# dmuley/sph-code

Measured on AMD Instinct MI355X. Metric: particle-steps/sec + achieved HBM GB/s, 10^6-particle 3D sphere, 1/2/4/8 GPUs, higher is better.
Workload: dtype f64

## Files before the change

sph-code_amd/csrc/sphx_api.hip:

```cpp
#include "sphx_internal.h"
#include <stdarg.h>
#include <stdlib.h>
#include <new>

int sphx_set_err(sphx_ctx* ctx, int code, const char* fmt, ...) {
    if (ctx) {
        va_list ap;
        va_start(ap, fmt);
        vsnprintf(ctx->err, sizeof(ctx->err), fmt, ap);
        va_end(ap);
    }
    return code;
}

void sphx_release(sphx_ctx* ctx, DevBuf& b) {
    for (size_t q = 0; q < ctx->allocs.size(); ++q)
        if (ctx->allocs[q] == b.p) { ctx->allocs[q] = ctx->allocs.back(); ctx->allocs.pop_back(); break; }
    if (b.p) (void)hipFree(b.p);
    b.p = nullptr;
    b.cap = 0;
}

int sphx_ensure(sphx_ctx* ctx, DevBuf& b, size_t bytes, hipStream_t in_use_on) {
    if (bytes == 0) bytes = 8;
    if (b.cap >= bytes) return SPHX_OK;
    if (b.p) {
        HIPCHK(hipStreamSynchronize(in_use_on));
        sphx_release(ctx, b);
    }
    size_t want = bytes + bytes / 8 + 256;
    hipError_t e = hipMalloc(&b.p, want);
    if (e != hipSuccess) {
        b.p = nullptr;
        return sphx_set_err(ctx, SPHX_E_NOMEM, "hipMalloc(%zu) failed: %s", want, hipGetErrorString(e));
    }
    b.cap = want;
    ctx->allocs.push_back(b.p);
    return SPHX_OK;
}

static void default_constants(sphx_constants* c) {
    c->k_B = 1.380649e-23;
    c->amu = 1.66053906892e-27;
    c->m_h = 1.0008 * c->amu;
    c->m_0 = 31.622776601683793 * 1.989e30;
    c->dt_0 = 60. * 60. * 24. * 365. * 250000.;
    c->max_age = 3e7 * 60. * 60. * 24. * 365.;
    c->pos_clamp = 1e11 * 149597870700.0;
    c->solar_luminosity = 3.846e26;
    c->c = 299792458.0;
}

extern "C" int sphx_version(void) { return 100; }

extern "C" const char* sphx_build_info(void) { return "gfx950 experiments=0"; }
extern "C" const char* sphx_tunables(const sphx_ctx* ctx) { return ctx ? ctx->tunables : ""; }

extern "C" int sphx_host_alloc(void** out, size_t bytes) {
    if (!out) return SPHX_E_ARG;
    *out = nullptr;
    if (bytes == 0) bytes = 8;
    if (hipHostMalloc(out, bytes, hipHostMallocDefault) != hipSuccess) {
        (void)hipGetLastError();
        *out = nullptr;
        return SPHX_E_NOMEM;
    }
    return SPHX_OK;
}
extern "C" int sphx_host_free(void* p) {
    if (p && hipHostFree(p) != hipSuccess) return SPHX_E_HIP;
    return SPHX_OK;
}

static hipError_t sphx_stream_create(hipStream_t* st, int side) {
    int least = 0, greatest = 0;
    if (hipDeviceGetStreamPriorityRange(&least, &greatest) != hipSuccess) return hipStreamCreateWithFlags(st, hipStreamNonBlocking);
    return hipStreamCreateWithPriority(st, hipStreamNonBlocking, side ? least : greatest);
}

extern "C" int sphx_create(sphx_ctx** out, int device) {
    if (!out) return SPHX_E_ARG;
    *out = nullptr;
    int count = 0;
    if (hipGetDeviceCount(&count) != hipSuccess || count <= 0 || device < 0 || device >= count) {
        fprintf(stderr, "sphx_create: no usable HIP device %d (found %d). libsphx has no CPU path.\n",
                device, count);
        return SPHX_E_HIP;
    }
    sphx_ctx* ctx = new (std::nothrow) sphx_ctx();
    if (!ctx) return SPHX_E_NOMEM;
    ctx->device = device;
    memset(&ctx->stats, 0, sizeof(ctx->stats));
    memset(&ctx->grid, 0, sizeof(ctx->grid));
    default_constants(&ctx->cst);
    auto env = [&](const char* name) -> const char* {
        const char* e = getenv(name);
        if (e) {
            const size_t used = strlen(ctx->tunables);
            snprintf(ctx->tunables + used, sizeof(ctx->tunables) - used, "%s%s=%s", used ? " " : "", name, e);
        }
        return e;
    };
    if (const char* e = env("SPHX_RSCALE")) { double v = atof(e); if (v >= 1.0) ctx->rscale = v; }
    if (const char* e = env("SPHX_CELL")) { double v = atof(e); if (v > 0.0) ctx->cell_factor = v; }
    if (const char* e = env("SPHX_RSCALE_BUILD")) { double v = atof(e); if (v >= 1.0) ctx->rscale_build = v; }
    if (const char* e = env("SPHX_VERLET")) ctx->use_verlet = atoi(e) != 0;
    if (const char* e = env("SPHX_BLOB")) ctx->use_blob = atoi(e) != 0;
    if (const char* e = env("SPHX_BLOB_CURVE")) ctx->blob_curve = atoi(e);
    if (const char* e = env("SPHX_KNN_GROUP")) ctx->use_group = atoi(e) != 0;
    if (const char* e = env("SPHX_HCLIP")) { double v = atof(e); if (v > 1.0) ctx->h_clip_factor = v; }
    if (const char* e = env("SPHX_TIMING_DETAIL")) ctx->timing_detail = atoi(e) != 0;
    if (const char* e = env("SPHX_MAX_CELLS")) { long long v = atoll(e); if (v > 0) ctx->max_cells = v; }
    if (const char* e = env("SPHX_CELL_FEEDBACK")) ctx->cell_feedback = atoi(e) != 0;
    if (const char* e = env("SPHX_CELL_FB_HI")) ctx->cell_fb_hi = atof(e);
    if (const char* e = env("SPHX_CELL_FB_LO")) ctx->cell_fb_lo = atof(e);
    if (const char* e = env("SPHX_DRAG_LDS")) ctx->drag_lds = atoi(e) != 0;
    if (const char* e = env("SPHX_BLOB_SPLIT")) ctx->blob_split_on = atoi(e) != 0;
    if (const char* e = env("SPHX_SPECIES_FUSED")) ctx->species_fused = atoi(e) != 0;
    if (const char* e = env("SPHX_SPECIES_LDS")) ctx->species_lds = atoi(e) != 0;
    if (const char* e = env("SPHX_HINT_DISTRUST")) ctx->distrust_mode = atoi(e);
    if (const char* e = env("SPHX_OUTLIER_LEVELS")) ctx->olev_mode = atoi(e);
    if (const char* e = env("SPHX_BOX_SIGMAS")) { double v = atof(e); if (v >= 1.0) ctx->box_sigmas = v; }
    if (const char* e = env("SPHX_GRAV_KERNEL")) ctx->grav_per_thread = atoi(e) == 0;
    if (const char* e = env("SPHX_GRAV_ORDER")) { int v = atoi(e); if (v == 1 || v == 2) ctx->grav_order = v; }
    if (const char* e = env("SPHX_GRAV_WS")) { int v = atoi(e); if (v >= 1 && v <= 4) ctx->grav_ws = v; }
    if (const char* e = env("SPHX_LDS")) ctx->use_lds = atoi(e) != 0;
    if (const char* e = env("SPHX_BLOB_SLOTS")) ctx->blob_slots = atoi(e);
    if (const char* e = env("SPHX_BLOB_WGS")) {
        int cus = 256;
        (void)hipDeviceGetAttribute(&cus, hipDeviceAttributeMultiprocessorCount, ctx->device);
        if (atoi(e) > 0) ctx->blob_grid = ((cus * atoi(e) + 7) / 8) * 8;
    }
    bool ok = hipSetDevice(device) == hipSuccess &&
              sphx_stream_create(&ctx->stream, 0) == hipSuccess &&
              hipHostMalloc((void**)&ctx->pinned, sizeof(PinnedLayout), hipHostMallocDefault) == hipSuccess;
    ctx->own_stream = ctx->stream;
    for (int i = 0; ok && i < 10; ++i) ok = hipEventCreate(&ctx->ev[i]) == hipSuccess;
    for (int r = 0; ok && r < 3; ++r)
        for (int i = 0; ok && i < 10; ++i) ok = hipEventCreate(&ctx->evring[r][i]) == hipSuccess;
    for (int r = 0; ok && r < 2; ++r)
        ok = hipEventCreateWithFlags(&ctx->lag_bev[r], hipEventDisableTiming) == hipSuccess &&
             hipEventCreateWithFlags(&ctx->lag_hev[r], hipEventDisableTiming) == hipSuccess;
    if (ok) ok = sphx_stream_create(&ctx->side_stream, 1) == hipSuccess &&
                 hipEventCreateWithFlags(&ctx->ev_join, hipEventDisableTiming) == hipSuccess &&
                 hipEventCreateWithFlags(&ctx->ev_perm, hipEventDisableTiming) == hipSuccess;
    if (ok) ok = sphx_ensure(ctx, ctx->scal, SC_NSLOTS * 8) == SPHX_OK &&
                 hipMemsetAsync(ctx->scal.p, 0, SC_NSLOTS * 8, ctx->stream) == hipSuccess &&
                 sphx_ensure(ctx, ctx->badc, (size_t)BADC_BUCKETS * BADC_STRIDE * sizeof(u64)) == SPHX_OK &&
                 hipMemsetAsync(ctx->badc.p, 0, (size_t)BADC_BUCKETS * BADC_STRIDE * sizeof(u64), ctx->stream) == hipSuccess;
    if (!ok) {
        fprintf(stderr, "sphx_create: HIP initialisation failed on device %d\n", device);
        delete ctx;
        return SPHX_E_HIP;
    }
    *out = ctx;
    return SPHX_OK;
}

extern "C" void sphx_destroy(sphx_ctx* ctx) {
    if (!ctx) return;
    (void)hipSetDevice(ctx->device);
    if (ctx->stream) (void)hipStreamSynchronize(ctx->stream);
    for (void* p : ctx->allocs) (void)hipFree(p);
    for (int i = 0; i < 10; ++i)
        if (ctx->ev[i]) (void)hipEventDestroy(ctx->ev[i]);
    for (StageTimer* t : {&ctx->arb_t, &ctx->rad_t, &ctx->cool_t})
        for (int i = 0; i < 5; ++i)
            if (t->ev[i]) (void)hipEventDestroy(t->ev[i]);
    for (int r = 0; r < 3; ++r)
        for (int i = 0; i < 10; ++i)
            if (ctx->evring[r][i]) (void)hipEventDestroy(ctx->evring[r][i]);
    for (int r = 0; r < 2; ++r) {
        if (ctx->lag_bev[r]) (void)hipEventDestroy(ctx->lag_bev[r]);
        if (ctx->lag_hev[r]) (void)hipEventDestroy(ctx->lag_hev[r]);
    }
    if (ctx->pinned) (void)hipHostFree(ctx->pinned);
    if (ctx->olev_ev) (void)hipEventDestroy(ctx->olev_ev);
    if (ctx->ev_join) (void)hipEventDestroy(ctx->ev_join);
    if (ctx->ev_perm) (void)hipEventDestroy(ctx->ev_perm);
    if (ctx->side_stream) (void)hipStreamDestroy(ctx->side_stream);
    if (ctx->own_stream) (void)hipStreamDestroy(ctx->own_stream);
    delete ctx;
}

extern "C" const char* sphx_last_error(const sphx_ctx* ctx) { return ctx ? ctx->err : "null context"; }

extern "C" int sphx_set_constants(sphx_ctx* ctx, const sphx_constants* c) {
    if (!ctx || !c) return SPHX_E_ARG;
    ctx->cst = *c;
    return SPHX_OK;
}
extern "C" int sphx_set_tuning(sphx_ctx* ctx, double rscale, double cell_factor) {
    if (!ctx) return SPHX_E_ARG;
    if (rscale > 0.0) {
        if (rscale < 1.0) return sphx_set_err(ctx, SPHX_E_ARG, "rscale %g < 1", rscale);
        ctx->rscale = rscale;
    }
    if (cell_factor > 0.0) ctx->cell_factor = cell_factor;
    return SPHX_OK;
}
extern "C" int sphx_set_incremental(sphx_ctx* ctx, int verlet, double rscale_build) {
    if (!ctx) return SPHX_E_ARG;
    ctx->use_verlet = verlet != 0;
    if (!ctx->use_verlet) ctx->list_valid = false;
    if (rscale_build > 0.0) {
        if (rscale_build < 1.0) return sphx_set_err(ctx, SPHX_E_ARG, "rscale_build %g < 1", rscale_build);
        ctx->rscale_build = rscale_build;
    }
    return SPHX_OK;
}
extern "C" int sphx_get_constants(const sphx_ctx* ctx, sphx_constants* c) {
    if (!ctx || !c) return SPHX_E_ARG;
    *c = ctx->cst;
    return SPHX_OK;
}

static int upload(sphx_ctx* ctx, DevBuf& b, const void* host, size_t bytes) {
    SPHX_TRY(sphx_ensure(ctx, b, bytes));
    HIPCHK(hipMemcpyAsync(b.p, host, bytes, hipMemcpyHostToDevice, ctx->stream));
    return SPHX_OK;
}
static int download(sphx_ctx* ctx, void* host, const void* dev, size_t bytes) {
    if (!host) return SPHX_OK;
    HIPCHK(hipMemcpyAsync(host, dev, bytes, hipMemcpyDeviceToHost, ctx->stream));
    return SPHX_OK;
}
int sphx_upload_f64(sphx_ctx* ctx, const CopyF64* t, int nt) {
    for (int i = 0; i < nt; ++i)
        if (t[i].host)
            HIPCHK(hipMemcpyAsync(const_cast<void*>(t[i].dev), t[i].host, t[i].count * sizeof(double), hipMemcpyHostToDevice, ctx->stream));
    return SPHX_OK;
}
int sphx_download_f64(sphx_ctx* ctx, const CopyF64* t, int nt) {
    for (int i = 0; i < nt; ++i)
        if (t[i].host && t[i].dev && t[i].count > 0)
            HIPCHK(hipMemcpyAsync(const_cast<void*>(t[i].host), t[i].dev, t[i].count * sizeof(double), hipMemcpyDeviceToHost, ctx->stream));
    return SPHX_OK;
}

int StageTimer::begin(sphx_ctx* ctx) {
    for (int i = 0; i < 5; ++i)
        if (!ev[i]) HIPCHK(hipEventCreate(&ev[i]));
    for (int i = 0; i < 4; ++i) ms[i] = 0.0;
    return mark(ctx, 0);
}
int StageTimer::mark(sphx_ctx* ctx, int i) {
    HIPCHK(hipEventRecord(ev[i], ctx->stream));
    return SPHX_OK;
}
int StageTimer::end(sphx_ctx* ctx) {
    for (int i = 0; i < 4; ++i) {
        float t = 0.f;
        HIPCHK(hipEventElapsedTime(&t, ev[i], ev[i + 1]));
        ms[i] = t;
    }
    return SPHX_OK;
}
static int last_timing(sphx_ctx* ctx, StageTimer sphx_ctx::*t, double ms[4]) {
    if (!ctx || !ms) return SPHX_E_ARG;
    for (int i = 0; i < 4; ++i) ms[i] = (ctx->*t).ms[i];
    return SPHX_OK;
}
extern "C" int sphx_arb_last_timing(sphx_ctx* ctx, double ms[4]) { return last_timing(ctx, &sphx_ctx::arb_t, ms); }
extern "C" int sphx_rad_last_timing(sphx_ctx* ctx, double ms[4]) { return last_timing(ctx, &sphx_ctx::rad_t, ms); }
extern "C" int sphx_cool_last_timing(sphx_ctx* ctx, double ms[4]) { return last_timing(ctx, &sphx_ctx::cool_t, ms); }

extern "C" int sphx_neighbors(sphx_ctx* ctx, int64_t n, int k, const double* points, double dist,
                              double eps, int64_t* idx, double* dist_out, int64_t* nontriv,
                              double* h) {
    (void)eps;
// ... 245 lines not shown
static int step_cell_hint(sphx_ctx* ctx, int64_t n, double* cell_hint) {
    *cell_hint = 0.0;
    if (ctx->step_count == 0) return SPHX_OK;
    const double* hs;
    if (ctx->lag_hvalid[ctx->lag_hslot]) {
        HIPCHK(hipEventSynchronize(ctx->lag_halias[ctx->lag_hslot] ? ctx->lag_halias[ctx->lag_hslot]
                                                                     : ctx->lag_hev[ctx->lag_hslot]));
        hs = ctx->pinned->lag[ctx->lag_hslot].hs;
        const u64* sv = (const u64*)hs;
        for (int q = 0; q < 10; ++q) ctx->knn_lag[q] = sv[(SC_NFAILQ - SC_HSUM) + q];
        ctx->knn_lag_valid = true;
    } else {
        HIPCHK(hipMemcpyAsync(ctx->pinned->hsum, ctx->scal.as<double>() + SC_HSUM, sizeof(ctx->pinned->hsum),
                              hipMemcpyDeviceToHost, ctx->stream));
        HIPCHK(hipStreamSynchronize(ctx->stream));
        hs = ctx->pinned->hsum;
    }
    const double hmean = hs[3] > 0.0 ? hs[0] / hs[3] : 0.0;
    if (hmean > 0.0 && isfinite(hmean)) {
        *cell_hint = ctx->cell_factor * sphx_cell_feedback(ctx, n) * hmean;
        ctx->h_clip = ctx->h_clip_factor * hmean;
    }
    return SPHX_OK;
}

static int step_search(sphx_ctx* ctx, int k, double dist, hipEvent_t* ev) {
    const int64_t n = ctx->n;
    if (ctx->use_verlet) SPHX_TRY(sphx_clamp(ctx, n, ctx->st));
    SPHX_TRY(sphx_ensure(ctx, ctx->nbr, (size_t)k * ctx->npad * sizeof(int)));
    if (ctx->use_verlet && ctx->list_valid && ctx->list_n == n && ctx->list_k == k) {
        StateArrays& r = ctx->st;
        HIPCHK(hipEventRecord(ev[1], ctx->stream));
        int64_t nfail = 0;
        SPHX_TRY(sphx_knn_refresh(ctx, n, k, r.x.as<double>(), r.y.as<double>(), r.z.as<double>(),
                                  ctx->nbr.as<int>(), r.hprev.as<double>(), &nfail));
        if (nfail == 0) {
            ctx->stats.refresh_steps++;
            return SPHX_OK;
        }
        ctx->list_valid = false;
    }
    double cell_hint = 0.0;
    SPHX_TRY(step_cell_hint(ctx, n, &cell_hint));
    {
        StateArrays& r = ctx->st;
        const bool blob = ctx->use_blob && !ctx->use_verlet;
        GridBuildOpts g;
        g.lagged = true;
        g.alias_ev = ev[1];
        g.sort_cells_later = blob;
        g.count_curve = blob && ctx->side_stream && ctx->ev_perm;
        if (!ctx->use_verlet) { g.clamp_vel[0] = r.vx.as<double>(); g.clamp_vel[1] = r.vy.as<double>(); g.clamp_vel[2] = r.vz.as<double>(); }
        SPHX_TRY(sphx_build_grid(ctx, n, k, r.x.as<double>(), r.y.as<double>(), r.z.as<double>(), cell_hint, g));
        if (blob) SPHX_TRY(sphx_build_blob_order(ctx, n, true));
    }
    const bool split = ctx->side_stream && !ctx->use_verlet;
    SPHX_TRY(sphx_permute_state(ctx, n, split, ev[1]));
    StateArrays& r = ctx->st;
    KnnIn in;
    in.xs = r.x.as<double>(); in.ys = r.y.as<double>(); in.zs = r.z.as<double>();
    in.id = r.id.as<int>(); in.inv = ctx->inv.as<int>();
    in.rsearch = r.hprev.as<double>();
    in.hinted = ctx->step_count > 0 && !ctx->use_verlet;
    in.lag_external = true;
    in.rscale = ctx->rscale;
    in.rbound = dist;
    KnnOut o;
    o.nbr = ctx->nbr.as<int>();
    o.h_sorted = r.hprev.as<double>();
    o.idx64 = nullptr; o.dist = nullptr; o.nontriv = nullptr; o.h_by_id = nullptr;
    if (ctx->use_verlet) {
        SPHX_TRY(sphx_ensure(ctx, ctx->list64, (size_t)n * 64 * sizeof(int)));
        SPHX_TRY(sphx_ensure(ctx, ctx->dref, (size_t)n * sizeof(double)));
        o.list64 = ctx->list64.as<int>();
        o.dref = ctx->dref.as<double>();
        in.rscale = ctx->rscale_build;
    }
    SPHX_TRY(sphx_knn(ctx, n, k, in, o));
    if (split) HIPCHK(hipStreamWaitEvent(ctx->stream, ctx->ev_perm, 0));
    if (ctx->use_verlet) {
        SPHX_TRY(sphx_save_list_positions(ctx, n, r.x.as<double>(), r.y.as<double>(), r.z.as<double>()));
        ctx->list_valid = true;
        ctx->list_n = n;
        ctx->list_k = k;
    }
    ctx->stats.rebuild_steps++;
    return SPHX_OK;
}

static int step_h_sums_out(sphx_ctx* ctx, int64_t n, const double* h, hipStream_t stream) {
    SPHX_TRY(sphx_hsum(ctx, n, h, stream));
    const int hsl = ctx->lag_hslot ^ 1;
    HIPCHK(hipMemcpyAsync(ctx->pinned->lag[hsl].hs, ctx->scal.as<double>() + SC_HSUM,
                          (SC_KGDBG + 2 - SC_HSUM + 1) * sizeof(double), hipMemcpyDeviceToHost, stream));
    HIPCHK(hipEventRecord(ctx->lag_hev[hsl], stream));
    ctx->lag_halias[hsl] = nullptr;
    ctx->lag_hvalid[hsl] = true;
    ctx->lag_hslot = hsl;
    return SPHX_OK;
}

static int step_sums(sphx_ctx* ctx, int k, hipEvent_t* ev, hipEvent_t search_end, bool detail) {
    const int64_t n = ctx->n;
    StateArrays& s = ctx->st;
    const bool pairwise = ctx->visc_mode == 1 && !ctx->loop_forms;
    const bool fork = ctx->qorder && ctx->use_lds && !ctx->loop_forms && ctx->side_stream;
    if (fork) HIPCHK(hipStreamWaitEvent(ctx->side_stream, search_end, 0));
    else SPHX_TRY(step_h_sums_out(ctx, n, s.hprev.as<double>(), ctx->stream));
    if (ctx->qorder && ctx->use_lds) SPHX_TRY(sphx_blob_translate(ctx, n, k));
    const bool species = ctx->s > 0 && ctx->fun_id.p;
    if (ctx->loop_forms) {
        if (ctx->drag || species)
            SPHX_TRY(sphx_prep(ctx, n, prep_in_of_state(s), pairwise, ctx->stream));
        if (detail) HIPCHK(hipEventRecord(ev[3], ctx->stream));
        SPHX_TRY(sphx_loop_step_sums(ctx, n, k, ctx->loop_d));
        if (detail) HIPCHK(hipEventRecord(ev[9], ctx->stream));
        if (species) SPHX_TRY(sphx_step_species(ctx, n, k));
        if (detail) HIPCHK(hipEventRecord(ev[4], ctx->stream));
        if (detail) HIPCHK(hipEventRecord(ev[5], ctx->stream));
    } else {
        SPHX_TRY(sphx_prep(ctx, n, prep_in_of_state(s), pairwise, fork ? ctx->side_stream : ctx->stream));
        if (fork) {
            HIPCHK(hipEventRecord(ctx->ev_join, ctx->side_stream));
            HIPCHK(hipStreamWaitEvent(ctx->stream, ctx->ev_join, 0));
            SPHX_TRY(step_h_sums_out(ctx, n, s.hprev.as<double>(), ctx->side_stream));
        }
        if (detail) HIPCHK(hipEventRecord(ev[3], ctx->stream));
        const bool sp_fused = species && ctx->species_fused && ctx->species_lds && ctx->use_lds && ctx->qorder && ctx->blob_lists &&
                              !ctx->map_perm && ctx->sp == 16 && ctx->s <= 16 && k <= SPHX_MAX_K;
        if (sp_fused) {
            const int S = ctx->s;
            SPHX_TRY(sphx_ensure(ctx, ctx->rho, (size_t)n * sizeof(double)));
            SPHX_TRY(sphx_ensure(ctx, ctx->rhod, (size_t)n * sizeof(double)));
            SPHX_TRY(sphx_ensure(ctx, ctx->nden, (size_t)n * sizeof(double)));
            SPHX_TRY(sphx_ensure(ctx, ctx->G, (size_t)n * 3 * sizeof(double)));
            SPHX_TRY(sphx_ensure(ctx, ctx->ha, (size_t)n * 3 * sizeof(double)));
            SPHX_TRY(sphx_ensure(ctx, ctx->F, (size_t)n * S * sizeof(double)));
            if (ctx->agb_on) {
                SPHX_TRY(sphx_ensure(ctx, ctx->Zmet, (size_t)n * sizeof(double)));
                SPHX_TRY(sphx_ensure(ctx, ctx->agb_dust, (size_t)n * S * sizeof(double)));
            }
            SPHX_TRY(sphx_blob_density_species(ctx, n, k, true, S, ctx->fun_id.as<double>(), s.id.as<int>(),
                                               s.m.as<double>(), ctx->F.as<double>(), ctx->Zmet.as<double>(),
                                               ctx->agb_dust.as<double>(), (ctx->agb_on && ctx->Zmet.p && ctx->agb_dust.p) ? 1 : 0));
        } else {
            SPHX_TRY(sphx_pass_density(ctx, n, k, true));
        }
        if (detail) HIPCHK(hipEventRecord(ev[9], ctx->stream));
        if (species && !sp_fused) SPHX_TRY(sphx_step_species(ctx, n, k));
        if (detail) HIPCHK(hipEventRecord(ev[4], ctx->stream));
        if (ctx->visc_mode == 1) {
            SPHX_TRY(sphx_pass_visc_pw(ctx, n, k, s.m.as<double>()));
        } else {
            SPHX_TRY(sphx_pass_pi(ctx, n, k, s.hprev.as<double>(), s.ptype.as<double>()));
            if (detail) HIPCHK(hipEventRecord(ev[5], ctx->stream));
            SPHX_TRY(sphx_pass_visc(ctx, n, k, s.m.as<double>()));
        }
    }
    if (ctx->drag)
        SPHX_TRY(sphx_pass_drag(ctx, n, k, s.m.as<double>(), s.ptype.as<double>(), s.mgm.as<double>(), s.mcs.as<double>()));
    return SPHX_OK;
}

static int one_step(sphx_ctx* ctx, int k, double dist, int first, double fixed_dt, bool call_first, bool call_last) {
    const int64_t n = ctx->n;
    const int ring = (int)(ctx->step_count % 3);
    hipEvent_t* ev = ctx->evring[ring];
    const bool detail = ctx->timing_detail;
    ctx->ev_detail[ring] = detail;
    const bool rec0 = detail || call_first, rec7 = detail || call_last;
    ctx->ev_has07[ring] = (rec0 ? 1 : 0) | (rec7 ? 2 : 0) | (ctx->visc_mode == 1 && !ctx->loop_forms ? 4 : 0);
    ctx->map_perm = nullptr;
    ctx->qorder = nullptr;
    ctx->blob_lists = false;
    ctx->blob_split_valid = false;
    ctx->pass_part = 0;
    ctx->nbr_api_valid = false;
    if (rec0) HIPCHK(hipEventRecord(ev[0], ctx->stream));
    SPHX_TRY(step_search(ctx, k, dist, ev));
    HIPCHK(hipEventRecord(ev[2], ctx->stream));
    SPHX_TRY(step_sums(ctx, k, ev, ev[2], detail));
    if (detail) HIPCHK(hipEventRecord(ev[6], ctx->stream));
    StateArrays& s = ctx->st;
    if (ctx->gravity) {
        SPHX_TRY(sphx_ensure(ctx, ctx->grav, (size_t)n * 3 * sizeof(double)));
        double* eps = ctx->scal.as<double>() + SC_GRAV_EPS;
        SPHX_TRY(sphx_median(ctx, n, s.hprev.as<double>(), eps));
        if (ctx->gravity == 1)
            SPHX_TRY(sphx_gravity_launch(ctx, n, s.x.as<double>(), s.y.as<double>(), s.z.as<double>(), 1,
                                         s.m.as<double>(), eps, 0.0, ctx->grav_G, nullptr, ctx->grav.as<double>()));
        else
            SPHX_TRY(sphx_gravity_tree_launch(ctx, n, s.x.as<double>(), s.y.as<double>(), s.z.as<double>(),
                                              s.m.as<double>(), ctx->grav_ws, eps, 0.0, ctx->grav_G, nullptr,
                                              ctx->grav.as<double>()));
    }
    if (detail) HIPCHK(hipEventRecord(ev[8], ctx->stream));
    SPHX_TRY(sphx_integrate(ctx, n, 1, first, fixed_dt));
    if (rec7) HIPCHK(hipEventRecord(ev[7], ctx->stream));
    ctx->step_count++;
    return SPHX_OK;
}

static int collect_stats(sphx_ctx* ctx, int ring) {
    if (!(ctx->ev_pending & (1u << ring))) return SPHX_OK;
    ctx->ev_pending &= ~(1u << ring);
    hipEvent_t* ev = ctx->evring[ring];
    const int has = ctx->ev_has07[ring];
    HIPCHK(hipEventSynchronize((has & 2) ? ev[7] : ev[2]));
    sphx_stats& st = ctx->stats;
    float ms[7] = {0.f, 0.f, 0.f, 0.f, 0.f, 0.f, 0.f};
    HIPCHK(hipEventElapsedTime(&ms[1], ev[1], ev[2]));
    st.ms_search += ms[1];
    st.steps += 1;
    st.search_steps += 1;
    st.n = ctx->n;
    if (!ctx->ev_detail[ring]) return SPHX_OK;
    float tot;
    HIPCHK(hipEventElapsedTime(&tot, ev[0], ev[7]));
    HIPCHK(hipEventElapsedTime(&ms[0], ev[0], ev[1]));
    st.ms_grid += ms[0]; st.ms_total += tot;
    for (int i = 2; i < 6; ++i) {
        if ((has & 4) && i >= 4) break;
        HIPCHK(hipEventElapsedTime(&ms[i], ev[i], ev[i + 1]));
    }
    if (has & 4) HIPCHK(hipEventElapsedTime(&ms[5], ev[4], ev[6]));
    st.ms_prep += ms[2];
    float mg = 0.f, mi = 0.f;
    HIPCHK(hipEventElapsedTime(&mg, ev[6], ev[8]));
    HIPCHK(hipEventElapsedTime(&mi, ev[8], ev[7]));
    ms[6] = mi;
    st.ms_gravity += mg;
    {
        float md = 0.f, msp = 0.f;
        HIPCHK(hipEventElapsedTime(&md, ev[3], ev[9]));
        HIPCHK(hipEventElapsedTime(&msp, ev[9], ev[4]));
        ms[3] = md;
        st.ms_species += msp;
    }
    st.ms_density += ms[3]; st.ms_pi += ms[4]; st.ms_visc += ms[5]; st.ms_integrate += ms[6];
    st.detail_steps += 1;
    return SPHX_OK;
}

extern "C" int sphx_step(sphx_ctx* ctx, int nsteps, int k, double dist, int first, double fixed_dt) {
    if (!ctx) return SPHX_E_ARG;
    if (!ctx->has_state) return sphx_set_err(ctx, SPHX_E_STATE, "sphx_step before sphx_state_upload");
    if (k < 1 || k > SPHX_MAX_K) return sphx_set_err(ctx, SPHX_E_ARG, "N_NEIGH=%d not in 1..%d", k, SPHX_MAX_K);
    if (nsteps < 1) return sphx_set_err(ctx, SPHX_E_ARG, "nsteps=%d < 1", nsteps);
    HIPCHK(hipSetDevice(ctx->device));
    if (!(dist > 0.0) || !isfinite(dist)) dist = 0.0;
    ctx->k = k;
    const bool per_call = !ctx->timing_detail;
    if (per_call) HIPCHK(hipEventRecord(ctx->ev[8], ctx->stream));
    for (int it = 0; it < nsteps; ++it) {
        const int ring = (int)(ctx->step_count % 3);
        SPHX_TRY(collect_stats(ctx, ring));
        SPHX_TRY(one_step(ctx, k, dist, first && it == 0, fixed_dt, false, false));
        ctx->ev_pending |= 1u << ring;
        SPHX_TRY(collect_stats(ctx, (ring + 1) % 3));
    }
    if (per_call) HIPCHK(hipEventRecord(ctx->ev[9], ctx->stream));
    HIPCHK(hipMemcpyAsync(ctx->pinned->scal, ctx->scal.p, SC_NSLOTS * 8, hipMemcpyDeviceToHost, ctx->stream));
    HIPCHK(hipStreamSynchronize(ctx->stream));
    for (int r = 0; r < 3; ++r) SPHX_TRY(collect_stats(ctx, (int)((ctx->step_count + r) % 3)));
    if (per_call) {
        float tot = 0.f;
        HIPCHK(hipEventElapsedTime(&tot, ctx->ev[8], ctx->ev[9]));
        ctx->stats.ms_total += tot;
    }
    const u64* sc = ctx->pinned->scal;
    memcpy(&ctx->dt_last, &sc[SC_DT], sizeof(double));
    ctx->stats.candidates = (int64_t)sc[SC_CAND];
    ctx->stats.retries = (int64_t)sc[SC_RETRY];
    ctx->stats.fallback_queries = (int64_t)(u32)sc[SC_NFAILQ];
    ctx->stats.short_rows = (int64_t)sc[SC_SHORT];
    SPHX_TRY(sphx_badc_read(ctx));
    return SPHX_OK;
}

extern "C" int sphx_state_download(sphx_ctx* ctx, double* pos, double* vel, double* accel,
                                   double* E_internal, double* T, double* sizes, double* rho,
                                   double* nden, double* visc_heat, double* dt_last) {
    if (!ctx) return SPHX_E_ARG;
    if (!ctx->has_state) return sphx_set_err(ctx, SPHX_E_STATE, "no state uploaded");
    HIPCHK(hipSetDevice(ctx->device));
    const int64_t n = ctx->n;
    const size_t nb = (size_t)n * sizeof(double);
    StateArrays& s = ctx->st;
    const int* id = s.id.as<int>();
    SPHX_TRY(sphx_ensure(ctx, ctx->out_a, 3 * nb));
    double* stage = ctx->out_a.as<double>();
    struct V3 { double* host; DevBuf *a, *b, *c; };
    V3 v3[] = {{pos, &s.x, &s.y, &s.z}, {vel, &s.vx, &s.vy, &s.vz}, {accel, &s.ax, &s.ay, &s.az}};
    for (V3& v : v3) {
        if (!v.host) continue;
        SPHX_TRY(sphx_soa3_to_aos_by_id(ctx, n, id, v.a->as<double>(), v.b->as<double>(), v.c->as<double>(), stage));
        SPHX_TRY(download(ctx, v.host, stage, 3 * nb));
        HIPCHK(hipStreamSynchronize(ctx->stream));
    }
    struct V1 { double* host; const double* dev; };
    const bool stepped = ctx->step_count > 0;
    V1 v1[] = {{E_internal, s.E.as<double>()}, {T, s.T.as<double>()}, {sizes, s.hprev.as<double>()},
               {rho, stepped ? ctx->rho.as<double>() : nullptr},
               {nden, stepped ? ctx->nden.as<double>() : nullptr},
               {visc_heat, stepped ? ctx->vh.as<double>() : nullptr}};
    for (V1& v : v1) {
        if (!v.host) continue;
        if (!v.dev) { memset(v.host, 0, nb); continue; }
        SPHX_TRY(sphx_scatter_rows_by_id(ctx, n, 1, id, v.dev, stage));
        SPHX_TRY(download(ctx, v.host, stage, nb));
        HIPCHK(hipStreamSynchronize(ctx->stream));
    }
    if (dt_last) *dt_last = ctx->dt_last;
    return SPHX_OK;
}

int sphx_agb_table_set(sphx_ctx* ctx, int S, int nspl, const int32_t* ntx, const int32_t* nty, const double* tx, const double* ty,
                       const double* coeffs, const int32_t* mapto, double divisor, const double* mu_specie, double solar_mass) {
    ctx->agb_on = false;
    if (nspl == 0) return SPHX_OK;
    if (S < 7 || S > AGB_MAX_SPEC) return sphx_set_err(ctx, SPHX_E_ARG, "AGB table: %d species (7..%d)", S, AGB_MAX_SPEC);
    if (!ntx || !nty || !tx || !ty || !coeffs || !mapto || !mu_specie)
        return sphx_set_err(ctx, SPHX_E_ARG, "AGB table: NULL argument");
    if (nspl < 1 || nspl > AGB_MAX_SPL) return sphx_set_err(ctx, SPHX_E_ARG, "AGB table: %d splines", nspl);
    if (!(divisor != 0.0)) return sphx_set_err(ctx, SPHX_E_ARG, "AGB table: divisor is 0");
    HIPCHK(hipSetDevice(ctx->device));
    AgbTable& t = ctx->agb;
    t.nspl = nspl; t.nspec = S;
// ... 155 lines not shown
```

sph-code_amd/csrc/sphx_blob.h:

```cpp
#pragma once
#include "sphx_internal.h"
#include "sphx_pair.h"
#include "sphx_settled.h"

#ifndef BLOB_P
#define BLOB_P 128
#endif
#define BLOB_T (2 * BLOB_P)
#define LPP SPHX_SUM_PARTS
#define PASS_T (BLOB_P * LPP)
#ifndef BLOB_S
#define BLOB_S 960
#endif
#ifndef DEDUP_PRIO
#define DEDUP_PRIO 2
#endif
#ifndef BLOB_STAGE_PRIO
#define BLOB_STAGE_PRIO 1
#endif
#ifndef PASS_MINW
#define PASS_MINW 4
#endif
#define BLOB_PROBES 96
#define SLOT_NONE 0xFFFFu
// ... 3 lines not shown
typedef unsigned short u16;

__device__ __forceinline__ Q4 lload4(const double2* img, int s, int c2) {
    const double2 lo = img[(2 * c2) * BLOB_S + s];
    const double2 hi = img[(2 * c2 + 1) * BLOB_S + s];
    return Q4{lo.x, lo.y, hi.x, hi.y};
}
struct Q8 { Q4 lo, hi; };
__device__ __forceinline__ Q8 lload8(const double2* img, int s) { return Q8{lload4(img, s, 0), lload4(img, s, 1)}; }
template <class Rec>
__device__ __forceinline__ Q8 gload8(const Rec* r) {
    const double* q = reinterpret_cast<const double*>(r);
    return Q8{gload4(q), gload4(q + 4)};
}
__device__ __forceinline__ double sqrt_mid(double x) {
    const double y = __builtin_amdgcn_rsq(x);
    double g = x * y;
    double h = 0.5 * y;
    const double r = __builtin_fma(-h, g, 0.5);
    g = __builtin_fma(g, r, g);
    h = __builtin_fma(h, r, h);
    const double d0 = __builtin_fma(-g, g, x);
    g = __builtin_fma(d0, h, g);
    const double d1 = __builtin_fma(-g, g, x);
    g = __builtin_fma(d1, h, g);
    return x > 0.0 ? g : 0.0;
}
struct SqrtMid { __device__ __forceinline__ double operator()(double x) const { return sqrt_mid(x); } };

__device__ __forceinline__ double pair_swap(double v) {
    const long long b = __double_as_longlong(v);
    const int lo = __builtin_amdgcn_update_dpp(0, (int)b, 0xB1, 0xF, 0xF, true);
    const int hi = __builtin_amdgcn_update_dpp(0, (int)(b >> 32), 0xB1, 0xF, 0xF, true);
    return __longlong_as_double(((long long)hi << 32) | (unsigned)lo);
}
__device__ __forceinline__ double pair_swap2(double v) {
    const long long b = __double_as_longlong(v);
    const int lo = __builtin_amdgcn_update_dpp(0, (int)b, 0x4E, 0xF, 0xF, true);
    const int hi = __builtin_amdgcn_update_dpp(0, (int)(b >> 32), 0x4E, 0xF, 0xF, true);
    return __longlong_as_double(((long long)hi << 32) | (unsigned)lo);
}
__device__ __forceinline__ double group_total(double acc) {
    acc = acc + pair_swap(acc);
    if (LPP == 4) acc = acc + pair_swap2(acc);
    return acc;
}
__device__ __forceinline__ double group_max(double v) {
    v = fmax(v, pair_swap(v));
    if (LPP == 4) v = fmax(v, pair_swap2(v));
    return v;
}
template <class S>
__device__ __forceinline__ void group_total_fields(S& s) {
    constexpr int NF = sizeof(S) / sizeof(double);
    static_assert(sizeof(S) == NF * sizeof(double), "a struct of doubles");
    double f[NF];
    __builtin_memcpy(f, &s, sizeof(S));
#pragma unroll
    for (int q = 0; q < NF; ++q) f[q] = group_total(f[q]);
    __builtin_memcpy(&s, f, sizeof(S));
}

#define NSTAGE ((BLOB_S + PASS_T - 1) / PASS_T)
#define NB (8 / LPP)
#define KPAD(k) ((((k) + 7) / 8) * 8)
#define IMG_BYTES(per_slot, k) ((size_t)BLOB_S * (per_slot) + (size_t)KPAD(k) * BLOB_P * sizeof(u16))

template <int NSIDE, class Rec>
__device__ __forceinline__ void stage(double2* img, double* side, u16* tile, const Rec* __restrict__ rec,
                                      const double* __restrict__ g0, int g0_stride,
                                      const double* __restrict__ g1, int g1_stride,
                                      const int* __restrict__ uq, const u16* __restrict__ slot16, int npad,
                                      int k, int b) {
    __builtin_amdgcn_s_setprio(BLOB_STAGE_PRIO);
    int ju[NSTAGE];
#pragma unroll
    for (int r = 0; r < NSTAGE; ++r) {
        const int s = threadIdx.x + r * PASS_T;
        ju[r] = (s < BLOB_S) ? uq[s] : -1;
    }
    const int pieces = KPAD(k) * (BLOB_P / 8);
    for (int q = threadIdx.x; q < pieces; q += PASS_T) {
        const int kk = q / (BLOB_P / 8), c = q % (BLOB_P / 8);
        uint4 v = make_uint4(0xFFFFFFFFu, 0xFFFFFFFFu, 0xFFFFFFFFu, 0xFFFFFFFFu);
        if (kk < k) v = *reinterpret_cast<const uint4*>(slot16 + (size_t)kk * npad + (size_t)b * BLOB_P + c * 8);
        *reinterpret_cast<uint4*>(tile + kk * BLOB_P + c * 8) = v;
    }
    double2 c[NSTAGE][4];
    double e0[NSTAGE], e1[NSTAGE];
#pragma unroll
    for (int r = 0; r < NSTAGE; ++r) {
        const int j = ju[r] < 0 ? 0 : ju[r];
        const double2* g = reinterpret_cast<const double2*>(&rec[j]);
        c[r][0] = g[0]; c[r][1] = g[1]; c[r][2] = g[2]; c[r][3] = g[3];
        e0[r] = (NSIDE > 0) ? g0[(size_t)j * g0_stride] : 0.0;
        e1[r] = (NSIDE > 1) ? g1[(size_t)j * g1_stride] : 0.0;
    }
#pragma unroll
    for (int r = 0; r < NSTAGE; ++r) {
        const int s = threadIdx.x + r * PASS_T;
        if (ju[r] >= 0) {
            if (NSIDE == 2) c[r][3].y = e0[r];
            img[0 * BLOB_S + s] = c[r][0]; img[1 * BLOB_S + s] = c[r][1];
            img[2 * BLOB_S + s] = c[r][2]; img[3 * BLOB_S + s] = c[r][3];
            if (NSIDE == 1) side[s] = e0[r];
            if (NSIDE == 2) side[s] = e1[r];
        }
    }
    __builtin_amdgcn_s_setprio(0);
}

__device__ __forceinline__ void load_slots(unsigned (&sl)[NB], const u16* tile, int m0, int half, int t) {
#pragma unroll
    for (int u = 0; u < NB; ++u) sl[u] = tile[(LPP * (m0 + u) + half) * BLOB_P + t];
}
__device__ __forceinline__ bool all_staged(const unsigned (&sl)[NB]) {
    unsigned worst = sl[0];
#pragma unroll
    for (int u = 1; u < NB; ++u) worst = worst > sl[u] ? worst : sl[u];
    return __ballot(worst >= SLOT_OVER) == 0ull;
}


struct BlobSel { const int* list; const int* cnt; int mode; };
__device__ __forceinline__ int blob_sel_count(const BlobSel& s, int nblk) {
    if (!s.list) return nblk;
    return (s.mode == 1) ? s.cnt[0] : (s.mode == 2) ? s.cnt[1] : s.cnt[0] + s.cnt[1];
}
__device__ __forceinline__ int blob_sel_at(const BlobSel& s, int bi, int count) {
    const int q = xcd_block(bi, count);
    return s.list ? s.list[q + (s.mode == 2 ? s.cnt[0] : 0)] : q;
}
BlobSel sphx_blob_sel(sphx_ctx* ctx, int part);

int sphx_blob_grid(sphx_ctx* ctx, int nblk);
int sphx_lds_opt_in(sphx_ctx* ctx, const void* kernel, size_t bytes);

#define BLOB_KERNEL __global__ __launch_bounds__(PASS_T, PASS_MINW) void
#define BLOB_COMMON int n, int npad, int k, int nblk, const int* __restrict__ nbr, const u16* __restrict__ slot16, \
                    const int* __restrict__ uniq, const int* __restrict__ qorder
template <class Kern, class... Rest>
static int blob_launch(sphx_ctx* ctx, Kern kern, int per_slot, size_t extra, int64_t n, int k, Rest... rest) {
    const int64_t npad = sphx_pad64(n);
    const int nblk = (int)((npad + BLOB_P - 1) / BLOB_P);
    SPHX_TRY(sphx_lds_opt_in(ctx, reinterpret_cast<const void*>(kern), IMG_BYTES(per_slot, SPHX_MAX_K) + extra));
    hipLaunchKernelGGL(kern, dim3(sphx_blob_grid(ctx, nblk)), dim3(PASS_T), IMG_BYTES(per_slot, k) + extra, ctx->stream, (int)n,
                       (int)npad, k, nblk, ctx->nbr.as<int>(), ctx->slot16.as<u16>(), ctx->uniq.as<int>(), ctx->qorder, rest...);
    HIPCHK(hipGetLastError());
    return SPHX_OK;
}

template <class P, class = void> struct BlobSettles { static constexpr bool value = false; };
template <class P> struct BlobSettles<P, decltype((void)P::SETTLES)> { static constexpr bool value = P::SETTLES; };
template <class P, class = void> struct BlobSaturates { static constexpr bool value = false; };
template <class P> struct BlobSaturates<P, decltype((void)P::SATURATES)> { static constexpr bool value = P::SATURATES; };
enum { BLOB_CNT_BLOBS_SETTLED = 0, BLOB_CNT_WAVES_SATURATED = 1 };
struct BlobSides { const double* g0 = nullptr; int s0 = 0; const double* g1 = nullptr; int s1 = 0; };

template <int NSIDE>
struct BlobLds {
    static __device__ __forceinline__ double2* img() { extern __shared__ double2 img[]; return img; }
    static __device__ __forceinline__ double* side() { return reinterpret_cast<double*>(img() + 4 * BLOB_S); }
    static __device__ __forceinline__ u16* tile() { return reinterpret_cast<u16*>(side() + (NSIDE ? BLOB_S : 0)); }
};

template <bool FAST, bool CLIP, class P>
__device__ __forceinline__ void blob_batch(const P& ps, typename P::Sums& a, double (&out)[NB], const unsigned (&sl)[NB],
                                           const int* __restrict__ jp, size_t colstep, const typename P::Row& row) {
    typedef BlobLds<P::NSIDE> L;
    typename P::Nb f[NB];
#pragma unroll
    for (int u = 0; u < NB; ++u) {
        if (FAST || sl[u] < SLOT_OVER) f[u] = ps.staged(L::img(), L::side(), (int)sl[u], jp + u * colstep);
        else if (sl[u] == SLOT_OVER) f[u] = ps.global(jp[u * colstep]);
        else f[u] = P::none(row);
    }
    if (FAST) __builtin_amdgcn_sched_barrier(0);
#pragma unroll
    for (int u = 0; u < NB; ++u) {
        out[u] = 0.0;
        if (!FAST && sl[u] == SLOT_NONE) continue;
        out[u] = ps.template term<CLIP>(a, f[u], row);
    }
}
template <class P>
__device__ __forceinline__ void blob_batch_any(const P& ps, int clip, typename P::Sums& a, double (&out)[NB],
                                               const unsigned (&sl)[NB], const int* __restrict__ jp, size_t colstep,
                                               const typename P::Row& row) {
    const bool fast = all_staged(sl);
    if constexpr (P::CLIPS) {
        if (fast && !clip) blob_batch<true, false>(ps, a, out, sl, jp, colstep, row);
        else if (fast) blob_batch<true, true>(ps, a, out, sl, jp, colstep, row);
        else if (!clip) blob_batch<false, false>(ps, a, out, sl, jp, colstep, row);
        else blob_batch<false, true>(ps, a, out, sl, jp, colstep, row);
    } else {
        if (fast) blob_batch<true, false>(ps, a, out, sl, jp, colstep, row);
        else blob_batch<false, false>(ps, a, out, sl, jp, colstep, row);
    }
}
template <bool FAST, class P>
__device__ __forceinline__ void blob_batch_short(const P& ps, double (&out)[NB], const unsigned (&sl)[NB],
                                                 const int* __restrict__ jp, size_t colstep, const typename P::Row& row) {
    typedef BlobLds<P::NSIDE> L;
    typename P::Vel f[NB];
#pragma unroll
    for (int u = 0; u < NB; ++u) {
        if (FAST || sl[u] < SLOT_OVER) f[u] = P::short_staged(L::img(), (int)sl[u]);
        else if (sl[u] == SLOT_OVER) f[u] = ps.short_global(jp[u * colstep]);
        else f[u] = P::short_none(row);
    }
#pragma unroll
    for (int u = 0; u < NB; ++u) {
        out[u] = 0.0;
        if (!FAST && sl[u] == SLOT_NONE) continue;
        out[u] = P::term_short(f[u], row);
    }
}
struct RowAhead { int i, o; unsigned first; double own; };
template <class P>
__device__ __forceinline__ RowAhead blob_row_ahead(const P& ps, int i, int p, int n, const u16* __restrict__ slot16,
                                                   const int* __restrict__ omap) {
    RowAhead r;
    r.i = i;
    r.o = (p < n) ? (omap ? omap[i] : i) : 0x7FFFFFFF;
    r.first = (p < n) ? slot16[p] : SLOT_NONE;
    r.own = ps.own(i);
    return r;
}
template <int T>
__device__ __forceinline__ bool block_all_at_barrier(bool mine, unsigned round) {
    __shared__ int verdict[2][T / 64];
    static_assert(T / 64 == 8, "eight waves: read as two 16-B pieces");
    int* v = verdict[round & 1];
    const int wave_all = __ballot(!mine) == 0ull;
    if ((threadIdx.x & 63) == 0) v[threadIdx.x >> 6] = wave_all;
    __syncthreads();
    const int4 lo = *reinterpret_cast<const int4*>(v), hi = *reinterpret_cast<const int4*>(v + 4);
    const int all = (lo.x & lo.y) & (lo.z & lo.w) & (hi.x & hi.y) & (hi.z & hi.w);
    return __builtin_amdgcn_readfirstlane(all) != 0;
}
template <int T>
__device__ __forceinline__ void block_add_count(unsigned v, u64* dst) {
    __shared__ unsigned sm[T / 64];
    if ((threadIdx.x & 63) == 0) sm[threadIdx.x >> 6] = v;
    __syncthreads();
    if (threadIdx.x == 0) {
        unsigned r = 0;
        for (int w = 0; w < T / 64; ++w) r += sm[w];
        if (r) atomicAdd(dst, (u64)r);
    }
}
template <class P>
__device__ __forceinline__ void blob_row_point(const P& ps, typename P::Row& row, const int* __restrict__ nbr, int p,
                                               int t) {
    typedef BlobLds<P::NSIDE> L;
    const unsigned sl0 = L::tile()[t];
    if (sl0 < SLOT_OVER) P::row_point(row, ps.staged(L::img(), L::side(), (int)sl0, nbr + p));
    else if (sl0 == SLOT_OVER) P::row_point(row, ps.global(nbr[p]));
}

template <class P>
__device__ __forceinline__ void blob_pass(const P& ps, int n, int npad, int k, int nblk, const int* __restrict__ nbr,
                                          const u16* __restrict__ slot16, const int* __restrict__ uniq,
                                          const int* __restrict__ qorder, int clip, const int* __restrict__ omap,
                                          int n_active, u64* ct_bits, const BlobSel& sel, u64* counts = nullptr) {
    static_assert(P::PER_SLOT == 64 + (P::NSIDE ? 8 : 0), "image bytes per slot: the record and one side value");
    constexpr bool SETTLES = BlobSettles<P>::value, SATURATES = BlobSaturates<P>::value;
    static_assert(!SATURATES || LPP == 4, "sphx_wave_saturated: a row's lanes are one nibble of the wave's mask");
    typedef BlobLds<P::NSIDE> L;
    const BlobSides sd = ps.sides();
    const int t = threadIdx.x / LPP, half = threadIdx.x & (LPP - 1);
    u64 my_ct = SPHX_CT_NONE;
    unsigned blobs_settled = 0, waves_saturated = 0;
    const int nsel = blob_sel_count(sel, nblk);
    const int stride = gridDim.x;
    auto particle_of = [&](int bq) -> int {
        const int pq = blob_sel_at(sel, bq, nsel) * BLOB_P + t;
        return (pq < n) ? qorder[pq] : 0;
    };
    auto nothing_left = [&](const RowAhead& r) -> bool {
        return !(r.o < n_active) || sphx_row_settled(r.own, r.first != SLOT_NONE, true);
    };
    RowAhead cur{0, 0x7FFFFFFF, SLOT_NONE, 0.0};
    int i_next = 0;
    bool blob_settled = false;
    unsigned round = 0;
    if constexpr (SETTLES) {
        if ((int)blockIdx.x < nsel)
            cur = blob_row_ahead(ps, particle_of(blockIdx.x), blob_sel_at(sel, blockIdx.x, nsel) * BLOB_P + t, n, slot16, omap);
        if ((int)blockIdx.x + stride < nsel) i_next = particle_of(blockIdx.x + stride);
        blob_settled = block_all_at_barrier<PASS_T>(nothing_left(cur), round++);
    }
    for (int bi = blockIdx.x; bi < nsel; bi += stride) {
        const int b = blob_sel_at(sel, bi, nsel);
        const int p = b * BLOB_P + t;
        int i, o;
        bool settled = false;
        auto fetch_ahead = [&]() {
            if constexpr (SETTLES) {
                if (bi + stride < nsel) {
                    cur = blob_row_ahead(ps, i_next, blob_sel_at(sel, bi + stride, nsel) * BLOB_P + t, n, slot16, omap);
                    if (bi + 2 * stride < nsel) i_next = particle_of(bi + 2 * stride);
                }
            }
        };
        if constexpr (SETTLES) {
            i = cur.i; o = cur.o;
            settled = sphx_row_settled(cur.own, cur.first != SLOT_NONE, o < n_active);
            if (blob_settled) {
                fetch_ahead();
                if (settled && !half) ps.settle(o);
                ++blobs_settled;
                blob_settled = block_all_at_barrier<PASS_T>(nothing_left(cur), round++);
                continue;
            }
        } else {
            i = (p < n) ? qorder[p] : 0;
        }
        stage<P::NSIDE>(L::img(), L::side(), L::tile(), ps.rec, sd.g0, sd.s0, sd.g1, sd.s1, uniq + (size_t)b * BLOB_S,
                        slot16, npad, k, b);
        typename P::Row row = ps.load_row(i);
        if constexpr (!SETTLES) o = (p < n) ? (omap ? omap[i] : i) : 0x7FFFFFFF;
        ps.load_out(row, o, o < n_active);
        if constexpr (SETTLES) fetch_ahead();
        __syncthreads();
        if (o < n_active) {
            if (SETTLES && __ballot(!settled) == 0ull) {
                if constexpr (SETTLES) { if (!half) ps.settle(o); }
            } else {
                if constexpr (P::ROW_FROM_LIST) blob_row_point(ps, row, nbr, p, t);
                typename P::Sums a{};
                double mx = 0.0;
                if (P::wanted(row)) {
                    const int nm = KPAD(k) / LPP;
                    unsigned sl[NB];
                    load_slots(sl, L::tile(), 0, half, t);
                    bool short_form = false;
                    bool short_used = false;
                    for (int m0 = 0; m0 < nm; m0 += NB) {
                        unsigned cur_sl[NB];
#pragma unroll
                        for (int u = 0; u < NB; ++u) cur_sl[u] = sl[u];
                        if (m0 + NB < nm) load_slots(sl, L::tile(), m0 + NB, half, t);
                        double out[NB];
                        const int* jp = nbr + ((size_t)(LPP * m0 + half) * npad + p);
                        if constexpr (SATURATES) {
                            if (__builtin_expect(short_form, false)) {
                                short_used = true;
                                if (all_staged(cur_sl)) blob_batch_short<true>(ps, out, cur_sl, jp, LPP * (size_t)npad, row);
                                else blob_batch_short<false>(ps, out, cur_sl, jp, LPP * (size_t)npad, row);
                            } else {
                                blob_batch_any(ps, clip, a, out, cur_sl, jp, LPP * (size_t)npad, row);
                                short_form = sphx_wave_saturated(__ballot(P::saturated(a)), __ballot(true));
                            }
                        } else {
                            blob_batch_any(ps, clip, a, out, cur_sl, jp, LPP * (size_t)npad, row);
                        }
                        if (P::VOTES) {
#pragma unroll
                            for (int u = 0; u < NB; ++u) mx = fmax(mx, out[u]);
                        }
                    }
                    if (SATURATES && short_used) ++waves_saturated;
                }
                group_total_fields(a);
                if (P::VOTES) mx = group_max(mx);
                if (!half) {
                    const u64 cb = ps.finish(a, mx, row, i, o);
                    my_ct = cb < my_ct ? cb : my_ct;
                }
            }
        }
        if constexpr (SETTLES) blob_settled = block_all_at_barrier<PASS_T>(nothing_left(cur), round++);
        else __syncthreads();
    }
    if (P::VOTES) block_min_vote<PASS_T>(my_ct, ct_bits);
    if constexpr (SETTLES) {
        if (counts && threadIdx.x == 0 && blobs_settled) atomicAdd(counts + BLOB_CNT_BLOBS_SETTLED, (u64)blobs_settled);
    }
    if constexpr (SATURATES) {
        if (counts) block_add_count<PASS_T>(waves_saturated, counts + BLOB_CNT_WAVES_SATURATED);
    }
}
```

sph-code_amd/csrc/sphx_blob.hip:

```cpp
#include "sphx_blob.h"
#include "sphx_wave.h"
#pragma clang fp contract(off)
#include <float.h>
#include <stdlib.h>
#include <stdio.h>
#ifndef BLOB_PI_SATURATES
#define BLOB_PI_SATURATES 1
#endif

#define DD_TAB 2048
#define DD_PROBES 64
__device__ __forceinline__ unsigned dd_hash(int j) { return ((unsigned)j * 2654435761u) >> 21; }

__global__ __launch_bounds__(BLOB_T) void blob_dedup_kernel(int n, int npad, int k, int slots,
                                                            const int* __restrict__ nbr, u16* slot16,
                                                            int* uniq, const int* __restrict__ qorder,
                                                            const int* __restrict__ omap, int n_active,
                                                            unsigned char* bclass) {
    __builtin_amdgcn_s_setprio(DEDUP_PRIO);
    extern __shared__ u16 dd_tile[];
    __shared__ int key[DD_TAB];
    __shared__ u16 slot_of[DD_TAB];
    __shared__ int wave_tot[BLOB_T / 64];
    const int b = xcd_block(blockIdx.x, gridDim.x);
    const int t = threadIdx.x >> 1, half = threadIdx.x & 1;
    const int p = b * BLOB_P + t;
    for (int q = threadIdx.x; q < DD_TAB; q += BLOB_T) key[q] = -1;
    __syncthreads();
    {
        const int nm = (k + 1) >> 1;
        const bool live = p < n;
        int jn[DD_BATCH];
#pragma unroll
        for (int u = 0; u < DD_BATCH; ++u) {
            const int kk = 2 * u + half;
            jn[u] = (kk < k && live) ? nbr[(size_t)kk * npad + p] : -1;
        }
        for (int m0 = 0; m0 < nm; m0 += DD_BATCH) {
            int jb[DD_BATCH];
#pragma unroll
            for (int u = 0; u < DD_BATCH; ++u) {
                jb[u] = jn[u];
                const int kk = 2 * (m0 + DD_BATCH + u) + half;
                jn[u] = (kk < k && live) ? nbr[(size_t)kk * npad + p] : -1;
            }
            unsigned hb[DD_BATCH];
            int eb[DD_BATCH];
#pragma unroll
            for (int u = 0; u < DD_BATCH; ++u) {
                hb[u] = dd_hash(jb[u] < 0 ? 0 : jb[u]);
                eb[u] = key[hb[u]];
            }
#pragma unroll
            for (int u = 0; u < DD_BATCH; ++u)
                if (jb[u] >= 0 && eb[u] == -1) {
                    const int old = atomicCAS(&key[hb[u]], -1, jb[u]);
                    eb[u] = (old == -1) ? jb[u] : old;
                }
#pragma unroll
            for (int u = 0; u < DD_BATCH; ++u) {
                const int kk = 2 * (m0 + u) + half;
                if (kk >= k) continue;
                const int j = jb[u];
                unsigned s = SLOT_NONE;
                if (j >= 0) {
                    unsigned h = hb[u];
                    s = SLOT_OVER;
                    if (eb[u] == j) {
                        s = h;
                    } else {
                        for (int probe = 1; probe < DD_PROBES; ++probe) {
                            h = (h + 1) & (DD_TAB - 1);
                            int e = key[h];
                            if (e == -1) {
                                e = atomicCAS(&key[h], -1, j);
                                if (e == -1) e = j;
                            }
                            if (e == j) { s = h; break; }
                        }
                    }
                }
                dd_tile[kk * BLOB_P + t] = (u16)s;
            }
        }
    }
    __syncthreads();
    constexpr int EPT = DD_TAB / BLOB_T;
    const int e0 = threadIdx.x * EPT;
    int cnt = 0;
#pragma unroll
    for (int q = 0; q < EPT; ++q) cnt += key[e0 + q] != -1;
    const int incl = wave_scan_incl(cnt);
    const int lane = threadIdx.x & 63, wv = threadIdx.x >> 6;
    if (lane == 63) wave_tot[wv] = incl;
    __syncthreads();
    int base = incl - cnt, total = 0;
#pragma unroll
    for (int w = 0; w < BLOB_T / 64; ++w) {
        const int tw = wave_tot[w];
        if (w < wv) base += tw;
        total += tw;
    }
    int* uq = uniq + (size_t)b * BLOB_S;
    int needs_ghost = 0;
#pragma unroll
    for (int q = 0; q < EPT; ++q) {
        const int j = key[e0 + q];
        if (j != -1) {
            slot_of[e0 + q] = (u16)(base < slots ? base : SLOT_OVER);
            if (base < slots) uq[base] = j;
            ++base;
            if (bclass && omap[j] >= n_active) needs_ghost = 1;
        }
    }
    for (int q = (total < slots ? total : slots) + threadIdx.x; q < BLOB_S; q += BLOB_T) uq[q] = -1;
    __syncthreads();
    const int pieces = k * (BLOB_P / 8);
    for (int q = threadIdx.x; q < pieces; q += BLOB_T) {
        u16* src = dd_tile + q * 8;
        const int kk = q / (BLOB_P / 8), c = q % (BLOB_P / 8);
        unsigned v[8];
#pragma unroll
        for (int u = 0; u < 8; ++u) {
            const unsigned e = src[u];
            v[u] = e < DD_TAB ? (unsigned)slot_of[e] : e;
            if (v[u] == SLOT_OVER) needs_ghost = 1;
        }
        if ((size_t)b * BLOB_P + c * 8 < (size_t)npad)
            *reinterpret_cast<uint4*>(slot16 + (size_t)kk * npad + (size_t)b * BLOB_P + c * 8) =
                make_uint4(v[0] | (v[1] << 16), v[2] | (v[3] << 16), v[4] | (v[5] << 16), v[6] | (v[7] << 16));
    }
    if (bclass) {
        const int owned_q = (half == 0 && p < n && omap[qorder[p]] < n_active) ? 1 : 0;
        const int any_owned = __syncthreads_or(owned_q);
        const int any_ghost = __syncthreads_or(needs_ghost);
        if (threadIdx.x == 0) bclass[b] = (unsigned char)(!any_owned ? 2 : (any_ghost ? 1 : 0));
    }
}

#define SPLIT_T 1024
__global__ __launch_bounds__(SPLIT_T) void blob_split_kernel(int nblk, const unsigned char* __restrict__ bclass, int* list,
                                                             int* cnt) {
    __shared__ int wsum[2][SPLIT_T / 64];
    const int per = (nblk + SPLIT_T - 1) / SPLIT_T;
    const int b0 = threadIdx.x * per, b1 = (b0 + per < nblk) ? b0 + per : nblk;
    int c0 = 0, c1 = 0;
    for (int b = b0; b < b1; ++b) { const int c = bclass[b]; c0 += c == 0; c1 += c == 1; }
    const int i0 = wave_scan_incl(c0), i1 = wave_scan_incl(c1);
    const int lane = threadIdx.x & 63, wv = threadIdx.x >> 6;
    if (lane == 63) { wsum[0][wv] = i0; wsum[1][wv] = i1; }
    __syncthreads();
    int o0 = i0 - c0, o1 = i1 - c1, t0 = 0, t1 = 0;
    for (int w = 0; w < SPLIT_T / 64; ++w) {
        if (w < wv) { o0 += wsum[0][w]; o1 += wsum[1][w]; }
        t0 += wsum[0][w]; t1 += wsum[1][w];
    }
    for (int b = b0; b < b1; ++b) {
        const int c = bclass[b];
        if (c == 0) list[o0++] = b;
        else if (c == 1) list[t0 + o1++] = b;
    }
    if (threadIdx.x == 0) { cnt[0] = t0; cnt[1] = t1; cnt[2] = nblk - t0 - t1; }
}

int sphx_blob_translate(sphx_ctx* ctx, int64_t n, int k) {
    const int64_t npad = sphx_pad64(n);
    const int nblk = (int)((npad + BLOB_P - 1) / BLOB_P);
    SPHX_TRY(sphx_ensure(ctx, ctx->slot16, (size_t)k * npad * sizeof(u16) + 512));
    SPHX_TRY(sphx_ensure(ctx, ctx->uniq, (size_t)nblk * BLOB_S * sizeof(int)));
    int slots = ctx->blob_slots;
    if (slots < 1) slots = 1;
    if (slots > BLOB_S) slots = BLOB_S;
    const bool split = ctx->map_perm != nullptr && ctx->blob_split_on;
    unsigned char* bclass = nullptr;
    ctx->blob_split_valid = false;
    if (split) {
        SPHX_TRY(sphx_ensure(ctx, ctx->blob_class, (size_t)nblk));
        SPHX_TRY(sphx_ensure(ctx, ctx->blob_split, ((size_t)nblk + 4) * sizeof(int)));
        bclass = ctx->blob_class.as<unsigned char>();
    }
    hipLaunchKernelGGL(blob_dedup_kernel, dim3(nblk), dim3(BLOB_T), (size_t)k * BLOB_P * sizeof(u16), ctx->stream, (int)n, (int)npad, k, slots,
                       ctx->nbr.as<int>(), ctx->slot16.as<u16>(), ctx->uniq.as<int>(), ctx->qorder, ctx->map_perm,
                       ctx->map_nactive, bclass);
    if (split) {
        int* list = ctx->blob_split.as<int>();
        hipLaunchKernelGGL(blob_split_kernel, dim3(1), dim3(SPLIT_T), 0, ctx->stream, nblk, bclass, list, list + (size_t)nblk);
        ctx->blob_split_valid = true;
        ctx->blob_split_nblk = nblk;
    }
    HIPCHK(hipGetLastError());
    ctx->blob_lists = true;
    return SPHX_OK;
}


struct DensityPass {
    typedef RecA Rec;
    typedef DensAcc Sums;
    static constexpr int NSIDE = 0, PER_SLOT = 64;
    static constexpr bool CLIPS = true, VOTES = false, ROW_FROM_LIST = true;
    const RecA* __restrict__ rec;
    double *rho_s, *rho, *rhod, *nden, *G, *ha;
    struct Row { double xr, yr, zr, hi2, ci, Ai; };
    typedef Q8 Nb;
    __device__ __forceinline__ BlobSides sides() const { return {}; }
    __device__ __forceinline__ Row load_row(int i) const {
        const Q8 s = gload8(&rec[i]);
        return Row{s.lo.a, s.lo.b, s.lo.c, s.lo.d, -6.0 * s.hi.a, s.hi.c};
    }
    __device__ __forceinline__ static void load_out(Row&, int, bool) {}
    __device__ __forceinline__ static void row_point(Row& r, const Nb& f) { r.xr = f.lo.a; r.yr = f.lo.b; r.zr = f.lo.c; }
    __device__ __forceinline__ static bool wanted(const Row&) { return true; }
    __device__ __forceinline__ Nb staged(const double2* img, const double*, int s, const int*) const {
        return lload8(img, s);
    }
    __device__ __forceinline__ Nb global(int j) const { return gload8(&rec[j]); }
    __device__ __forceinline__ static Nb none(const Row& r) { return Nb{Q4{r.xr, r.yr, r.zr, 0.0}, Q4{0.0, 0.0, 0.0, 0.0}}; }
    template <bool CLIP>
    __device__ __forceinline__ double term(Sums& a, const Nb& f, const Row& r) const {
        return density_term<SqrtMid>(a, f.lo, f.hi, r.xr, r.yr, r.zr, r.hi2, r.ci, r.Ai, CLIP);
    }
    __device__ __forceinline__ u64 finish(const Sums& a, double, const Row&, int i, int o) const {
        rho[o] = a.rho; rhod[o] = a.rd; nden[o] = a.n;
        rho_s[i] = a.rho;
        if (G) { G[3 * (size_t)o + 0] = -a.gx; G[3 * (size_t)o + 1] = -a.gy; G[3 * (size_t)o + 2] = -a.gz; }
        ha[3 * (size_t)o + 0] = -a.gx / a.rho;
        ha[3 * (size_t)o + 1] = -a.gy / a.rho;
        ha[3 * (size_t)o + 2] = -a.gz / a.rho;
        return SPHX_CT_NONE;
    }
};
BLOB_KERNEL blob_density_kernel(BLOB_COMMON, int clip, const int* __restrict__ omap, int n_active,
                                const RecA* __restrict__ rec, double* rho_s, double* rho, double* rhod, double* nden,
                                double* G, double* ha, BlobSel sel) {
    blob_pass(DensityPass{rec, rho_s, rho, rhod, nden, G, ha}, n, npad, k, nblk, nbr, slot16, uniq, qorder, clip, omap,
              n_active, nullptr, sel);
}

struct PiPass {
    typedef RecB Rec;
    struct Sums { double pi; };
    static constexpr int NSIDE = 1, PER_SLOT = 72;
    static constexpr bool CLIPS = false, VOTES = true, ROW_FROM_LIST = true;
    static constexpr bool SATURATES = BLOB_PI_SATURATES != 0;
    const RecB* __restrict__ rec;
    const double* __restrict__ rho_s;
    const RecSelf* __restrict__ selfr;
    RecBC* bc;
    double *Pi, *BwOut;
    struct Row { Q4 r0, rv; double rho_i, cs_i, ms_i, h_i; };
    struct Nb { Q8 q; double rho; };
    __device__ __forceinline__ BlobSides sides() const { return {rho_s, 1}; }
    __device__ __forceinline__ Row load_row(int i) const {
        const RecSelf sf = selfr[i];
        const Q8 s = gload8(&rec[i]);
        return Row{s.lo, s.hi, rho_s[i], sf.csi, sf.mg, sf.h};
    }
    __device__ __forceinline__ static void load_out(Row&, int, bool) {}
    __device__ __forceinline__ static void row_point(Row& r, const Nb& f) { r.r0 = f.q.lo; r.rv = f.q.hi; }
    __device__ __forceinline__ static bool wanted(const Row&) { return true; }
    __device__ __forceinline__ Nb staged(const double2* img, const double* side, int s, const int*) const {
        return Nb{lload8(img, s), side[s]};
    }
    __device__ __forceinline__ Nb global(int j) const { return Nb{gload8(&rec[j]), rho_s[j]}; }
    __device__ __forceinline__ static Nb none(const Row& r) { return Nb{Q8{r.r0, r.rv}, r.rho_i}; }
    template <bool CLIP>
    __device__ __forceinline__ double term(Sums& a, const Nb& f, const Row& r) const {
        const PiPair t = pi_term<SqrtMid>(f.q.lo, f.q.hi, f.rho, r.r0, r.rv, r.rho_i, r.cs_i);
        a.pi += t.pi;
        return t.rel;
    }
    typedef Q4 Vel;
    __device__ __forceinline__ static bool saturated(const Sums& a) { return sphx_is_nan(a.pi); }
    __device__ __forceinline__ static Vel short_staged(const double2* img, int s) { return lload4(img, s, 1); }
    __device__ __forceinline__ Vel short_global(int j) const { return gload4(reinterpret_cast<const double*>(&rec[j]) + 4); }
    __device__ __forceinline__ static Vel short_none(const Row& r) { return r.rv; }
    __device__ __forceinline__ static double term_short(const Vel& qv, const Row& r) { return pi_rel(qv, r.rv); }
    __device__ __forceinline__ u64 finish(const Sums& a, double maxrel, const Row& r, int i, int o) const {
        Pi[o] = a.pi;
        const double bw = fmax(r.ms_i, 0.0) * a.pi;
        bc[i].Bw = bw;
        if (BwOut) BwOut[o] = bw;
        return (r.ms_i > 0.0) ? ct_vote_bits(r.h_i, maxrel) : SPHX_CT_NONE;
    }
};
BLOB_KERNEL blob_pi_kernel(BLOB_COMMON, const int* __restrict__ omap, int n_active, const RecB* __restrict__ recb,
                           const double* __restrict__ rho_s, const RecSelf* __restrict__ selfr, RecBC* bc, double* Pi,
                           double* BwOut, u64* ct_bits, BlobSel sel, u64* counts) {
    blob_pass(PiPass{recb, rho_s, selfr, bc, Pi, BwOut}, n, npad, k, nblk, nbr, slot16, uniq, qorder, 0, omap, n_active,
              ct_bits, sel, counts);
}

struct ViscPass {
    typedef RecB Rec;
    typedef ViscAcc Sums;
    static constexpr int NSIDE = 2, PER_SLOT = 72;
    static constexpr bool CLIPS = true, VOTES = false, ROW_FROM_LIST = true;
    static constexpr bool SETTLES = true;
    const RecB* __restrict__ rec;
    const RecBC* __restrict__ bc;
    const double* __restrict__ m;
    double *va, *vh;
    struct Row { Q4 r0, rv; double hi2, ci, Bi, mi; };
    struct Nb { Q8 q; double c1; };
    __device__ __forceinline__ BlobSides sides() const {
        const double* bcd = reinterpret_cast<const double*>(bc);
        return {bcd, 2, bcd + 1, 2};
    }
    __device__ __forceinline__ Row load_row(int i) const {
        const double2 bci = *reinterpret_cast<const double2*>(&bc[i]);
        const Q8 s = gload8(&rec[i]);
        return Row{s.lo, s.hi, s.lo.d, -6.0 * bci.y, bci.x, 0.0};
    }
    __device__ __forceinline__ void load_out(Row& r, int o, bool on) const { r.mi = on ? m[o] : 0.0; }
    __device__ __forceinline__ static void row_point(Row& r, const Nb& f) { r.r0 = f.q.lo; r.rv = f.q.hi; }
    __device__ __forceinline__ static bool wanted(const Row&) { return true; }
    __device__ __forceinline__ Nb staged(const double2* img, const double* side, int s, const int*) const {
        return Nb{lload8(img, s), side[s]};
    }
    __device__ __forceinline__ Nb global(int j) const {
        Nb f{gload8(&rec[j]), 0.0};
        const double2 tt = *reinterpret_cast<const double2*>(&bc[j]);
        f.q.hi.d = tt.x; f.c1 = tt.y;
        return f;
    }
    __device__ __forceinline__ static Nb none(const Row& r) { return Nb{Q8{r.r0, r.rv}, 0.0}; }
    template <bool CLIP>
    __device__ __forceinline__ double term(Sums& a, const Nb& f, const Row& r) const {
        visc_term<SqrtMid>(a, f.q.lo, f.q.hi, f.q.hi.d, f.c1, r.r0, r.rv, r.hi2, r.ci, r.Bi, CLIP);
        return 0.0;
    }
    __device__ __forceinline__ u64 finish(const Sums& a, double, const Row& r, int, int o) const {
        va[3 * (size_t)o + 0] = -a.x; va[3 * (size_t)o + 1] = -a.y; va[3 * (size_t)o + 2] = -a.z;
        vh[o] = a.h * r.mi / 2.0;
        return SPHX_CT_NONE;
    }
    __device__ __forceinline__ double own(int i) const { return bc[i].Bw; }
    __device__ __forceinline__ void settle(int o) const {
        const double q = __builtin_nan("");
        va[3 * (size_t)o + 0] = q; va[3 * (size_t)o + 1] = q; va[3 * (size_t)o + 2] = q;
        vh[o] = q;
    }
};
BLOB_KERNEL blob_visc_kernel(BLOB_COMMON, int clip, const int* __restrict__ omap, int n_active,
                             const RecB* __restrict__ recb, const RecBC* __restrict__ bc, const double* __restrict__ m,
                             double* va, double* vh, BlobSel sel, u64* counts) {
    blob_pass(ViscPass{recb, bc, m, va, vh}, n, npad, k, nblk, nbr, slot16, uniq, qorder, clip, omap, n_active, nullptr, sel,
              counts);
}

struct ViscPwPass {
    typedef RecB Rec;
    typedef ViscAcc Sums;
    static constexpr int NSIDE = 1, PER_SLOT = 72;
    static constexpr bool CLIPS = true, VOTES = true, ROW_FROM_LIST = true;
    const RecB* __restrict__ rec;
    const double* __restrict__ rho_s;
    const RecBC* __restrict__ bc;
    const RecSelf* __restrict__ selfr;
    const double* __restrict__ m;
    double *va, *vh;
    struct Row { Q4 r0, rv; double rho_i, cs_i, h_i, mg, hi2, ci, mi; };
    struct Nb { Q8 q; double rho, mc; };
    __device__ __forceinline__ BlobSides sides() const { return {rho_s, 1}; }
    __device__ __forceinline__ Row load_row(int i) const {
        const RecSelf sf = selfr[i];
        const double rho_i = rho_s[i], mci = bc[i].Bw;
        const Q8 s = gload8(&rec[i]);
        return Row{s.lo, s.hi, rho_i, sf.csi, sf.h, sf.mg, s.lo.d, -6.0 * mci, 0.0};
    }
    __device__ __forceinline__ void load_out(Row& r, int o, bool on) const { r.mi = on ? m[o] : 0.0; }
    __device__ __forceinline__ static void row_point(Row& r, const Nb& f) { r.r0 = f.q.lo; r.rv = f.q.hi; }
    __device__ __forceinline__ static bool wanted(const Row&) { return true; }
    __device__ __forceinline__ Nb staged(const double2* img, const double* side, int s, const int* jp) const {
        return Nb{lload8(img, s), side[s], bc[*jp].Bw};
    }
    __device__ __forceinline__ Nb global(int j) const { return Nb{gload8(&rec[j]), rho_s[j], bc[j].Bw}; }
    __device__ __forceinline__ static Nb none(const Row& r) { return Nb{Q8{r.r0, r.rv}, r.rho_i, 0.0}; }
    template <bool CLIP>
    __device__ __forceinline__ double term(Sums& a, const Nb& f, const Row& r) const {
        return visc_pw_term<SqrtMid>(a, f.q.lo, f.q.hi, f.rho, f.mc, r.r0, r.rv, r.rho_i, r.cs_i, r.hi2, r.ci, CLIP);
    }
    __device__ __forceinline__ u64 finish(const Sums& a, double maxrel, const Row& r, int, int o) const {
        va[3 * (size_t)o + 0] = -a.x; va[3 * (size_t)o + 1] = -a.y; va[3 * (size_t)o + 2] = -a.z;
        vh[o] = a.h * r.mi / 2.0;
        return (r.mg > 0.0) ? ct_vote_bits(r.h_i, maxrel) : SPHX_CT_NONE;
    }
};
BLOB_KERNEL blob_visc_pw_kernel(BLOB_COMMON, int clip, const int* __restrict__ omap, int n_active,
                                const RecB* __restrict__ recb, const double* __restrict__ rho_s,
                                const RecBC* __restrict__ bc, const RecSelf* __restrict__ selfr,
                                const double* __restrict__ m, double* va, double* vh, u64* ct_bits, BlobSel sel) {
    blob_pass(ViscPwPass{recb, rho_s, bc, selfr, m, va, vh}, n, npad, k, nblk, nbr, slot16, uniq, qorder, clip, omap, n_active,
              ct_bits, sel);
}

template <int SPEC_MAXM>
__device__ __forceinline__ void species_sweeps(const double (&w)[SPEC_MAXM], double2* img, const u16* tile,
                                               const int* __restrict__ uq, const int* __restrict__ nbr, int n, int npad,
                                               int nm, int p, int i, int t, int half, bool live, int S,
                                               const double* __restrict__ fun, const int* __restrict__ row_of,
                                               const double* __restrict__ m, const AgbTable& agb, int agb_on, double* F,
                                               double* Zout, double* agb_out) {
    double tot[16];
#pragma unroll
    for (int hh = 0; hh < 2; ++hh) {
        __syncthreads();
        {
            int ju[NSTAGE];
#pragma unroll
            for (int r = 0; r < NSTAGE; ++r) {
                const int s = threadIdx.x + r * PASS_T;
                ju[r] = (s < BLOB_S) ? uq[s] : -1;
            }
            double2 c[NSTAGE][4];
#pragma unroll
            for (int r = 0; r < NSTAGE; ++r) {
                const int jr = ju[r] < 0 ? 0 : ju[r];
                const double2* g = reinterpret_cast<const double2*>(fun + (size_t)(row_of ? row_of[jr] : jr) * 16) + 4 * hh;
                c[r][0] = g[0]; c[r][1] = g[1]; c[r][2] = g[2]; c[r][3] = g[3];
            }
#pragma unroll
            for (int r = 0; r < NSTAGE; ++r) {
                const int s = threadIdx.x + r * PASS_T;
                if (ju[r] >= 0) {
                    img[0 * BLOB_S + s] = c[r][0]; img[1 * BLOB_S + s] = c[r][1];
                    img[2 * BLOB_S + s] = c[r][2]; img[3 * BLOB_S + s] = c[r][3];
                }
            }
        }
        __syncthreads();
        double acc[8];
#pragma unroll
        for (int q = 0; q < 8; ++q) acc[q] = 0.0;
#pragma unroll
        for (int mm = 0; mm < SPEC_MAXM; ++mm) {
            if (mm < nm) {
                const unsigned sl = tile[(LPP * mm + half) * BLOB_P + t];
                if (sl != SLOT_NONE && live) {
                    Q4 f0, f1;
                    if (sl < SLOT_OVER) { f0 = lload4(img, (int)sl, 0); f1 = lload4(img, (int)sl, 1); }
                    else {
                        const int jo = nbr[(size_t)(LPP * mm + half) * npad + p];
                        const double* q = fun + (size_t)(row_of ? row_of[jo] : jo) * 16 + 8 * hh;
                        f0 = gload4(q); f1 = gload4(q + 4);
                    }
                    const double wm = w[mm];
                    acc[0] += wm * f0.a; acc[1] += wm * f0.b; acc[2] += wm * f0.c; acc[3] += wm * f0.d;
                    acc[4] += wm * f1.a; acc[5] += wm * f1.b; acc[6] += wm * f1.c; acc[7] += wm * f1.d;
                }
            }
        }
#pragma unroll
        for (int q = 0; q < 8; ++q) tot[8 * hh + q] = group_total(acc[q]);
    }
    if (live && !half) {
#pragma unroll
        for (int q = 0; q < 16; ++q)
            if (q < S) F[(size_t)q * n + i] = tot[q];
    }
    if (live && agb_on) {
        const double Z = species_metallicity(agb, tot, S);
        if (!half) Zout[i] = Z;
        const double Mi = m[i];
        double* row = agb_out + (size_t)i * S;
        for (int q = half; q < S; q += LPP)
            if (!((agb.covered >> q) & 1u)) row[q] = 0.0;
        for (int o = half; o < agb.nspl; o += LPP) {
            double val;
            const int target = agb_one_spline(agb, o, Mi, Z, val);
            if (target >= 0) row[target] = val;
        }
    }
}

template <int SPEC_MAXM>
__global__ __launch_bounds__(PASS_T, PASS_MINW) void blob_density_species_kernel(int n, int npad, int k, int nblk,
        const int* __restrict__ nbr, const u16* __restrict__ slot16, const int* __restrict__ uniq,
        const int* __restrict__ qorder, int clip, const RecA* __restrict__ rec, double* rho_s, double* rho, double* rhod,
        double* nden, double* G, double* ha,
        int S, const double* __restrict__ fun, const int* __restrict__ row_of, const double* __restrict__ m, AgbTable agb,
        int agb_on, double* F, double* Zout, double* agb_out) {
    const DensityPass ps{rec, rho_s, rho, rhod, nden, G, ha};
    double2* img = BlobLds<0>::img();
    u16* tile = BlobLds<0>::tile();
    const int t = threadIdx.x / LPP, half = threadIdx.x & (LPP - 1);
    const int nm = KPAD(k) / LPP;
    for (int bi = blockIdx.x; bi < nblk; bi += gridDim.x) {
        const int b = xcd_block(bi, nblk);
        const int p = b * BLOB_P + t;
        const bool live = p < n;
        const int i = live ? qorder[p] : 0;
        const int* uq = uniq + (size_t)b * BLOB_S;
        stage<0>(img, nullptr, tile, rec, nullptr, 0, nullptr, 0, uq, slot16, npad, k, b);
        DensityPass::Row row = ps.load_row(i);
        __syncthreads();
        double w[SPEC_MAXM];
#pragma unroll
        for (int mm = 0; mm < SPEC_MAXM; ++mm) w[mm] = 0.0;
        if (live) {
            blob_row_point(ps, row, nbr, p, t);
// ... 70 lines not shown
        }
        species_sweeps(w, img, tile, uq, nbr, n, npad, nm, p, i, t, half, live, S, fun, row_of, m, agb, agb_on, F, Zout, agb_out);
        __syncthreads();
    }
}

#define DRAG_XLDS (BLOB_S * (2 * sizeof(int) + 1))
template <bool FILL>
__global__ __launch_bounds__(PASS_T, PASS_MINW) void blob_drag_kernel(int n, int npad, int k, int nblk,
                                                           const int* __restrict__ nbr,
                                                           const u16* __restrict__ slot16,
                                                           const int* __restrict__ uniq,
                                                           const int* __restrict__ qorder,
                                                           const RecB* __restrict__ recb,
                                                           const double* __restrict__ m,
                                                           const double* __restrict__ ptype,
                                                           const double* __restrict__ mgm,
                                                           const double* __restrict__ mcs,
                                                           const int* __restrict__ id, double* onto, DragScatter sc) {
    extern __shared__ double2 img[];
    u16* tile = reinterpret_cast<u16*>(img + (FILL ? 4 * BLOB_S : 0));
    int* cntL = reinterpret_cast<int*>(tile + KPAD(k) * BLOB_P);
    int* baseL = cntL + BLOB_S;
    unsigned char* dust = reinterpret_cast<unsigned char*>(baseL + BLOB_S);
    const int t = threadIdx.x / LPP, part = threadIdx.x & (LPP - 1);
    const int nm = KPAD(k) / LPP;
    for (int bi = blockIdx.x; bi < nblk; bi += gridDim.x) {
        const int b = xcd_block(bi, nblk);
        const int p = b * BLOB_P + t;
        const bool live = p < n;
        const int i = live ? qorder[p] : 0;
        const int* uq = uniq + (size_t)b * BLOB_S;
        if (FILL) {
            stage<0>(img, nullptr, tile, recb, nullptr, 0, nullptr, 0, uq, slot16, npad, k, b);
        } else {
            const int pieces = KPAD(k) * (BLOB_P / 8);
            for (int q = threadIdx.x; q < pieces; q += PASS_T) {
                const int kk = q / (BLOB_P / 8), c = q % (BLOB_P / 8);
                uint4 v = make_uint4(0xFFFFFFFFu, 0xFFFFFFFFu, 0xFFFFFFFFu, 0xFFFFFFFFu);
                if (kk < k) v = *reinterpret_cast<const uint4*>(slot16 + (size_t)kk * npad + (size_t)b * BLOB_P + c * 8);
                *reinterpret_cast<uint4*>(tile + kk * BLOB_P + c * 8) = v;
            }
        }
        for (int s = threadIdx.x; s < BLOB_S; s += PASS_T) {
            const int j = uq[s];
            dust[s] = (j >= 0 && ptype[j] == 2.0) ? 1 : 0;
            cntL[s] = 0;
        }
        __syncthreads();
        if (live) {
            for (int m0 = 0; m0 < nm; ++m0) {
                const int kk = LPP * m0 + part;
                const unsigned sl = tile[kk * BLOB_P + t];
                if (sl < SLOT_OVER) {
                    if (dust[sl] && uq[sl] != i) atomicAdd(&cntL[sl], 1);
                } else if (sl == SLOT_OVER && !FILL) {
                    const int j = nbr[(size_t)kk * npad + p];
                    if (j != i && ptype[j] == 2.0) atomicAdd(&sc.cnt[j], 1);
                }
            }
        }
        __syncthreads();
        if (!FILL) {
            for (int s = threadIdx.x; s < BLOB_S; s += PASS_T)
                if (cntL[s]) atomicAdd(&sc.cnt[uq[s]], cntL[s]);
            __syncthreads();
            continue;
        }
        for (int s = threadIdx.x; s < BLOB_S; s += PASS_T) {
            const int c = cntL[s];
            if (c) {
                const int j = uq[s];
                baseL[s] = sc.start[j] + atomicSub(&sc.cnt[j], c) - c;
                cntL[s] = 0;
            }
        }
        const double* rq = reinterpret_cast<const double*>(&recb[i]);
        const Q4 r0 = gload4(rq), rv = gload4(rq + 4);
        __syncthreads();
        double ox = 0.0, oy = 0.0, oz = 0.0;
        if (live) {
            unsigned dm = 0;
            for (int m0 = 0; m0 < nm; ++m0) {
                const int kk = LPP * m0 + part;
                const unsigned sl = tile[kk * BLOB_P + t];
                bool d = false;
                if (sl < SLOT_OVER) d = dust[sl] != 0;
                else if (sl == SLOT_OVER) d = ptype[nbr[(size_t)kk * npad + p]] == 2.0;
                dm |= (d ? 1u : 0u) << m0;
            }
            while (dm) {
                const int m0 = __builtin_ctz(dm);
                dm &= dm - 1;
                const int kk = LPP * m0 + part;
                const unsigned sl = tile[kk * BLOB_P + t];
                int j;
                Q4 q0, qv;
                if (sl < SLOT_OVER) {
                    j = uq[sl];
                    q0 = lload4(img, (int)sl, 0); qv = lload4(img, (int)sl, 1);
                } else {
                    j = nbr[(size_t)kk * npad + p];
                    const double* qb = reinterpret_cast<const double*>(&recb[j]);
                    q0 = gload4(qb); qv = gload4(qb + 4);
                }
                const Vec3 f = drag_term(ox, oy, oz, q0, qv, r0, rv, j, m, mgm, mcs);
                if (j != i) {
                    const int slot = (sl < SLOT_OVER) ? baseL[sl] + atomicAdd(&cntL[sl], 1)
                                                      : sc.start[j] + atomicSub(&sc.cnt[j], 1) - 1;
                    sphx_drag_put(sc, slot, ((u64)(unsigned)id[i] << 8) | (u64)kk, -f.x, -f.y, -f.z);
                }
            }
        }
        const double tx = group_total(ox), ty = group_total(oy), tz = group_total(oz);
        if (live && part == 0) { onto[3 * (size_t)i] = tx; onto[3 * (size_t)i + 1] = ty; onto[3 * (size_t)i + 2] = tz; }
        __syncthreads();
    }
}

BlobSel sphx_blob_sel(sphx_ctx* ctx, int part) {
    if (!ctx->blob_split_valid) return BlobSel{nullptr, nullptr, 0};
    const int* list = ctx->blob_split.as<int>();
    return BlobSel{list, list + (size_t)ctx->blob_split_nblk, part == 0 ? 3 : part};
}

int sphx_blob_grid(sphx_ctx* ctx, int nblk) {
    if (ctx->blob_grid <= 0) {
        int cus = 256;
        (void)hipDeviceGetAttribute(&cus, hipDeviceAttributeMultiprocessorCount, ctx->device);
        ctx->blob_grid = ((cus * 2 + 7) / 8) * 8;
    }
    return nblk < ctx->blob_grid ? nblk : ctx->blob_grid;
}

int sphx_lds_opt_in(sphx_ctx* ctx, const void* kernel, size_t bytes) {
    for (int q = 0; q < ctx->n_lds_raised; ++q)
        if (ctx->lds_raised[q] == kernel) return SPHX_OK;
    if (ctx->n_lds_raised == SPHX_LDS_KERNELS)
        return sphx_set_err(ctx, SPHX_E_HIP, "sphx_lds_opt_in: more than %d kernels", SPHX_LDS_KERNELS);
    HIPCHK(hipFuncSetAttribute(kernel, hipFuncAttributeMaxDynamicSharedMemorySize, (int)bytes));
    ctx->lds_raised[ctx->n_lds_raised++] = kernel;
    return SPHX_OK;
}

static int blob_n_active(const sphx_ctx* ctx, int64_t n) { return ctx->map_perm ? ctx->map_nactive : (int)n; }

int sphx_blob_density(sphx_ctx* ctx, int64_t n, int k, bool lean) {
    return blob_launch(ctx, blob_density_kernel, DensityPass::PER_SLOT, 0, n, k, ctx->clip_grad, ctx->map_perm,
                       blob_n_active(ctx, n), ctx->rec1.as<RecA>(), ctx->rho_s.as<double>(), ctx->rho.as<double>(),
                       ctx->rhod.as<double>(), ctx->nden.as<double>(), lean ? nullptr : ctx->G.as<double>(), ctx->ha.as<double>(),
                       sphx_blob_sel(ctx, ctx->pass_part));
}

int sphx_blob_pi(sphx_ctx* ctx, int64_t n, int k, u64* ct_bits) {
    return blob_launch(ctx, blob_pi_kernel, PiPass::PER_SLOT, 0, n, k, ctx->map_perm, blob_n_active(ctx, n), ctx->recv.as<RecB>(),
                       ctx->rho_s.as<double>(), ctx->self_s.as<RecSelf>(), ctx->bc_s.as<RecBC>(), ctx->Pi.as<double>(),
                       ctx->map_perm ? ctx->Bw.as<double>() : nullptr, ct_bits, sphx_blob_sel(ctx, ctx->pass_part),
                       ctx->scal.as<u64>() + SC_SETTLED);
}

int sphx_blob_visc(sphx_ctx* ctx, int64_t n, int k, const double* m) {
    return blob_launch(ctx, blob_visc_kernel, ViscPass::PER_SLOT, 0, n, k, ctx->clip_grad, ctx->map_perm, blob_n_active(ctx, n),
                       ctx->recv.as<RecB>(), ctx->bc_s.as<RecBC>(), m, ctx->va.as<double>(), ctx->vh.as<double>(),
                       sphx_blob_sel(ctx, ctx->pass_part), ctx->scal.as<u64>() + SC_SETTLED);
}

int sphx_blob_visc_pw(sphx_ctx* ctx, int64_t n, int k, const double* m, u64* ct_bits) {
    return blob_launch(ctx, blob_visc_pw_kernel, ViscPwPass::PER_SLOT, 0, n, k, ctx->clip_grad, ctx->map_perm,
                       blob_n_active(ctx, n), ctx->recv.as<RecB>(), ctx->rho_s.as<double>(), ctx->bc_s.as<RecBC>(),
                       ctx->self_s.as<RecSelf>(), m, ctx->va.as<double>(), ctx->vh.as<double>(), ct_bits, sphx_blob_sel(ctx, ctx->pass_part));
}

int sphx_blob_density_species(sphx_ctx* ctx, int64_t n, int k, bool lean, int S, const double* fun, const int* row_of,
                              const double* m_sorted, double* F, double* Z, double* agb, int agb_on) {
    const auto kern = (KPAD(k) / LPP <= 10) ? blob_density_species_kernel<10> : blob_density_species_kernel<16>;
    return blob_launch(ctx, kern, 64, 0, n, k, ctx->clip_grad, ctx->rec1.as<RecA>(), ctx->rho_s.as<double>(), ctx->rho.as<double>(),
                       ctx->rhod.as<double>(), ctx->nden.as<double>(), lean ? nullptr : ctx->G.as<double>(),
                       ctx->ha.as<double>(), S, fun, row_of, m_sorted, ctx->agb, agb_on, F, Z, agb);
}

int sphx_blob_species(sphx_ctx* ctx, int64_t n, int k, int S, const double* fun, const int* row_of, const double* m_sorted, double* F,
                      double* Z, double* agb, int agb_on) {
    const auto kern = (KPAD(k) / LPP <= 10) ? blob_species_kernel<10> : blob_species_kernel<16>;
    return blob_launch(ctx, kern, 64, 0, n, k, S, ctx->rec1.as<RecA>(), fun, row_of, m_sorted, ctx->agb, agb_on, F, Z, agb);
}

int sphx_blob_drag(sphx_ctx* ctx, int64_t n, int k, bool count_only, const double* m, const double* ptype, const double* mgm,
                   const double* mcs, const int* id, double* onto, const DragScatter& sc) {
    if (count_only)
        return blob_launch(ctx, blob_drag_kernel<false>, 0, DRAG_XLDS, n, k, nullptr, m, ptype, mgm, mcs, id, onto, sc);
    return blob_launch(ctx, blob_drag_kernel<true>, 64, DRAG_XLDS, n, k, ctx->recv.as<RecB>(), m, ptype, mgm, mcs, id, onto, sc);
}
```

sph-code_amd/csrc/sphx_dev.hip:

```cpp
#include "sphx_internal.h"
#pragma clang fp contract(off)
#include <float.h>
#include "sphx_leapfrog.h"

extern "C" int sphx_set_stream(sphx_ctx* ctx, void* stream) {
    if (!ctx) return SPHX_E_ARG;
    HIPCHK(hipSetDevice(ctx->device));
    HIPCHK(hipStreamSynchronize(ctx->stream));
    ctx->stream = (hipStream_t)stream;
    return SPHX_OK;
}

extern "C" int sphx_reset_stream(sphx_ctx* ctx) {
    if (!ctx) return SPHX_E_ARG;
    HIPCHK(hipSetDevice(ctx->device));
    HIPCHK(hipStreamSynchronize(ctx->stream));
    ctx->stream = ctx->own_stream;
    return SPHX_OK;
}

__global__ __launch_bounds__(256) void gather3_aos_kernel(int n, const int* perm, const double* aos,
                                                          double* xs, double* ys, double* zs, int* inv) {
    int t = blockIdx.x * blockDim.x + threadIdx.x;
    if (t >= n) return;
    const int p = perm[t];
    xs[t] = aos[3 * (size_t)p]; ys[t] = aos[3 * (size_t)p + 1]; zs[t] = aos[3 * (size_t)p + 2];
    if (inv) inv[p] = t;
}

__global__ __launch_bounds__(256) void inject_field_kernel(int n, const int* perm, const double* src,
                                                           double* dst, int stride) {
    int t = blockIdx.x * blockDim.x + threadIdx.x;
    if (t >= n) return;
    dst[(size_t)t * stride] = src[perm[t]];
}

int sphx_dev_collect(sphx_ctx* ctx) {
    if (!ctx->dev_ev_pending) return SPHX_OK;
    ctx->dev_ev_pending = false;
    HIPCHK(hipEventSynchronize(ctx->ev[2]));
    float ms = 0.f;
    HIPCHK(hipEventElapsedTime(&ms, ctx->ev[1], ctx->ev[2]));
    ctx->stats.ms_search += ms;
    ctx->stats.steps += 1;
    ctx->stats.search_steps += 1;
    ctx->stats.n = ctx->map_nactive;
    return SPHX_OK;
}

extern "C" int sphx_dev_search(sphx_ctx* ctx, int64_t n_total, int64_t n_owned, int k, const double* pos,
                               const double* hint, double rscale, double dist, double* h_out) {
    if (!ctx) return SPHX_E_ARG;
    NEED(pos); NEED(h_out);
    if (n_total < 1 || n_total > 0x7FFFFFF0ll || n_owned < 0 || n_owned > n_total)
        return sphx_set_err(ctx, SPHX_E_ARG, "n_total=%lld n_owned=%lld out of range", (long long)n_total,
                            (long long)n_owned);
    if (k < 1 || k > SPHX_MAX_K) return sphx_set_err(ctx, SPHX_E_ARG, "N_NEIGH=%d not in 1..%d", k, SPHX_MAX_K);
    HIPCHK(hipSetDevice(ctx->device));
    SPHX_TRY(sphx_dev_collect(ctx));
    const int64_t n = n_total;
    const size_t nb = (size_t)n * sizeof(double);
    ctx->map_perm = nullptr;
    ctx->qorder = nullptr;
    ctx->gx_built = false;
    DevBuf* bufs[] = {&ctx->in_b, &ctx->in_c, &ctx->in_d, &ctx->in_e, &ctx->in_f, &ctx->in_g};
    for (DevBuf* b : bufs) SPHX_TRY(sphx_ensure(ctx, *b, nb));
    double *x = ctx->in_b.as<double>(), *y = ctx->in_c.as<double>(), *z = ctx->in_d.as<double>();
    double *xs = ctx->in_e.as<double>(), *ys = ctx->in_f.as<double>(), *zs = ctx->in_g.as<double>();
    SPHX_TRY(sphx_aos_to_soa3(ctx, n, pos, x, y, z));
    double cell_hint = 0.0;
    if (ctx->dev_hmean > 0.0) cell_hint = ctx->cell_factor * sphx_cell_feedback(ctx, n) * ctx->dev_hmean;
    GridBuildOpts gopts;
    gopts.lagged = true;
    SPHX_TRY(sphx_build_grid(ctx, n, k, x, y, z, cell_hint, gopts));
    hipLaunchKernelGGL(gather3_aos_kernel, dim3((unsigned)((n + 255) / 256)), dim3(256), 0, ctx->stream,
                       (int)n, ctx->perm.as<int>(), pos, xs, ys, zs, (int*)nullptr);
    HIPCHK(hipGetLastError());
    SPHX_TRY(sphx_ensure(ctx, ctx->nbr, (size_t)k * sphx_pad64(n) * sizeof(int)));
    ctx->map_perm = ctx->perm.as<int>();
    ctx->qorder = nullptr;
    ctx->blob_lists = false;
    ctx->blob_split_valid = false;
    ctx->pass_part = 0;
    if (ctx->use_blob) SPHX_TRY(sphx_build_blob_order(ctx, n));
    ctx->map_nactive = (int)n_owned;
    ctx->n = n;
    ctx->npad = sphx_pad64(n);
    ctx->k = k;
    KnnOut o;
    o.nbr = ctx->nbr.as<int>();
    o.h_sorted = nullptr; o.idx64 = nullptr; o.dist = nullptr; o.nontriv = nullptr;
    o.h_by_id = h_out;
    KnnIn in;
    in.xs = xs; in.ys = ys; in.zs = zs;
    in.id = ctx->perm.as<int>(); in.inv = ctx->inv.as<int>();
    in.rsearch = hint;
    in.hinted = in.hint_by_id = (hint != nullptr);
    in.rscale = rscale > 0.0 ? rscale : ctx->rscale;
    in.rbound = dist;
    HIPCHK(hipEventRecord(ctx->ev[1], ctx->stream));
    int rc = sphx_knn(ctx, n, k, in, o);
    HIPCHK(hipEventRecord(ctx->ev[2], ctx->stream));
    ctx->dev_ev_pending = (rc == SPHX_OK);
    if (rc == SPHX_OK && ctx->qorder && ctx->use_lds) rc = sphx_blob_translate(ctx, n, k);
    return rc;
}

extern "C" int sphx_dev_get_order(sphx_ctx* ctx, int64_t n_total, int32_t* out) {
    if (!ctx) return SPHX_E_ARG;
    NEED(out);
    if (!ctx->map_perm || ctx->n != n_total)
        return sphx_set_err(ctx, SPHX_E_STATE, "sphx_dev_get_order: no search over %lld particles", (long long)n_total);
    HIPCHK(hipSetDevice(ctx->device));
    HIPCHK(hipMemcpyAsync(out, ctx->map_perm, (size_t)n_total * sizeof(int), hipMemcpyDeviceToDevice, ctx->stream));
    return SPHX_OK;
}

extern "C" int sphx_dev_select_blobs(sphx_ctx* ctx, int part) {
    if (!ctx) return SPHX_E_ARG;
    if (part < 0 || part > 2) return sphx_set_err(ctx, SPHX_E_ARG, "sphx_dev_select_blobs: part %d not in 0..2", part);
    ctx->pass_part = 0;
    if (part == 0) return 0;
    if (!(ctx->map_perm && ctx->qorder && ctx->blob_lists && ctx->blob_split_valid)) return 0;
    ctx->pass_part = part;
    return 1;
}

extern "C" int sphx_dev_blob_split_counts(sphx_ctx* ctx, int32_t counts[3]) {
    if (!ctx) return SPHX_E_ARG;
    NEED(counts);
    if (!ctx->blob_split_valid) return sphx_set_err(ctx, SPHX_E_STATE, "sphx_dev_blob_split_counts: no split (LDS passes off, or no search yet)");
    HIPCHK(hipSetDevice(ctx->device));
    HIPCHK(hipMemcpyAsync(counts, ctx->blob_split.as<int>() + (size_t)ctx->blob_split_nblk, 3 * sizeof(int),
                          hipMemcpyDeviceToHost, ctx->stream));
    HIPCHK(hipStreamSynchronize(ctx->stream));
    return SPHX_OK;
}

extern "C" int sphx_dev_set_mean_h(sphx_ctx* ctx, double mean_h) {
    if (!ctx) return SPHX_E_ARG;
    ctx->dev_hmean = mean_h;
    return SPHX_OK;
}

extern "C" int sphx_dev_prep(sphx_ctx* ctx, const double* pos, const double* vel, const double* mass,
                             const double* h, const double* T, const double* mu, const double* gamma,
                             const double* ptype) {
    if (!ctx) return SPHX_E_ARG;
    NEED(pos); NEED(vel); NEED(mass); NEED(h); NEED(T); NEED(mu); NEED(gamma); NEED(ptype);
    if (!ctx->map_perm) return sphx_set_err(ctx, SPHX_E_STATE, "sphx_dev_prep before sphx_dev_search");
    HIPCHK(hipSetDevice(ctx->device));
    PrepIn in;
    in.pos_aos(pos); in.vel_aos(vel);
    in.m = mass; in.h = h; in.T = T; in.mu = mu; in.gam = gamma; in.ptype = ptype;
    return sphx_prep(ctx, ctx->n, in, ctx->visc_mode == 1, ctx->stream);
}

struct Borrow {
    DevBuf& b;
    DevBuf saved;
    Borrow(DevBuf& buf, void* p, size_t bytes) : b(buf), saved(buf) {
        if (p) { b.p = p; b.cap = bytes; }
    }
    ~Borrow() { b = saved; }
    Borrow(const Borrow&) = delete;
    Borrow& operator=(const Borrow&) = delete;
};

extern "C" int sphx_dev_density(sphx_ctx* ctx, double* rho, double* rho_dust, double* nden,
                                double* hydro_accel) {
    if (!ctx) return SPHX_E_ARG;
    if (!ctx->map_perm) return sphx_set_err(ctx, SPHX_E_STATE, "sphx_dev_density before sphx_dev_search");
    HIPCHK(hipSetDevice(ctx->device));
    const size_t nb = (size_t)ctx->n * sizeof(double);
    Borrow b1(ctx->rho, rho, nb), b2(ctx->rhod, rho_dust, nb), b3(ctx->nden, nden, nb), b4(ctx->ha, hydro_accel, 3 * nb);
    SPHX_TRY(sphx_pass_density(ctx, ctx->n, ctx->k));
    return SPHX_OK;
}

extern "C" int sphx_dev_pi(sphx_ctx* ctx, const double* rho_complete, double* Pi, double* Bw, double* ct_out) {
    if (!ctx) return SPHX_E_ARG;
    NEED(rho_complete);
    if (!ctx->map_perm) return sphx_set_err(ctx, SPHX_E_STATE, "sphx_dev_pi before sphx_dev_search");
    HIPCHK(hipSetDevice(ctx->device));
    const int64_t n = ctx->n;
    if (ctx->pass_part != 1)
        hipLaunchKernelGGL(inject_field_kernel, dim3((unsigned)((n + 255) / 256)), dim3(256), 0, ctx->stream, (int)n,
                           ctx->map_perm, rho_complete, ctx->rho_s.as<double>(), 1);
    HIPCHK(hipGetLastError());
    if (ctx->pass_part == 2) ctx->ct_primed = true;
    {
        Borrow b1(ctx->Pi, Pi, (size_t)n * sizeof(double)), b2(ctx->Bw, Bw, (size_t)n * sizeof(double));
        SPHX_TRY(sphx_pass_pi(ctx, n, ctx->k, nullptr, nullptr));
    }
    if (ct_out)
        HIPCHK(hipMemcpyAsync(ct_out, ctx->scal.as<u64>() + SC_CT_BITS, 8, hipMemcpyDeviceToDevice, ctx->stream));
    return SPHX_OK;
}

extern "C" int sphx_dev_visc(sphx_ctx* ctx, const double* Bw_complete, const double* mass,
                             double* visc_accel, double* visc_heat) {
    if (!ctx) return SPHX_E_ARG;
    NEED(Bw_complete); NEED(mass);
    if (!ctx->map_perm) return sphx_set_err(ctx, SPHX_E_STATE, "sphx_dev_visc before sphx_dev_search");
    HIPCHK(hipSetDevice(ctx->device));
    const int64_t n = ctx->n;
    if (ctx->pass_part != 1)
        hipLaunchKernelGGL(inject_field_kernel, dim3((unsigned)((n + 255) / 256)), dim3(256), 0, ctx->stream, (int)n,
                           ctx->map_perm, Bw_complete, ctx->bc_s.as<double>(), 2);
    HIPCHK(hipGetLastError());
    Borrow b1(ctx->va, visc_accel, 3 * (size_t)n * sizeof(double)), b2(ctx->vh, visc_heat, (size_t)n * sizeof(double));
    SPHX_TRY(sphx_pass_visc(ctx, n, ctx->k, mass));
    return SPHX_OK;
}

extern "C" int sphx_dev_visc_pairwise(sphx_ctx* ctx, const double* rho_complete, const double* mass,
                                      double* visc_accel, double* visc_heat, double* ct_out) {
    if (!ctx) return SPHX_E_ARG;
    NEED(rho_complete); NEED(mass);
    if (!ctx->map_perm) return sphx_set_err(ctx, SPHX_E_STATE, "sphx_dev_visc_pairwise before sphx_dev_search");
    if (ctx->visc_mode != 1) return sphx_set_err(ctx, SPHX_E_STATE, "sphx_dev_visc_pairwise needs sphx_set_visc_mode(ctx, 1)");
    if (!ctx->recs_pw)
        return sphx_set_err(ctx, SPHX_E_STATE, "sphx_dev_visc_pairwise: the records were not built in pairwise mode "
                                               "(sphx_set_visc_mode(ctx, 1) before sphx_dev_prep)");
    HIPCHK(hipSetDevice(ctx->device));
    const int64_t n = ctx->n;
    if (ctx->pass_part != 1)
        hipLaunchKernelGGL(inject_field_kernel, dim3((unsigned)((n + 255) / 256)), dim3(256), 0, ctx->stream, (int)n,
                           ctx->map_perm, rho_complete, ctx->rho_s.as<double>(), 1);
    HIPCHK(hipGetLastError());
    if (ctx->pass_part == 2) ctx->ct_primed = true;
    {
        Borrow b1(ctx->va, visc_accel, 3 * (size_t)n * sizeof(double)), b2(ctx->vh, visc_heat, (size_t)n * sizeof(double));
        SPHX_TRY(sphx_pass_visc_pw(ctx, n, ctx->k, mass));
    }
    if (ct_out)
        HIPCHK(hipMemcpyAsync(ct_out, ctx->scal.as<u64>() + SC_CT_BITS, 8, hipMemcpyDeviceToDevice, ctx->stream));
    return SPHX_OK;
}

#define nan_to_num_v sphx_nan_to_num
struct DevIntegArgs {
    int n;
    double *pos, *vel, *acc, *E, *T;
    const double *m, *mu, *gam, *ptype, *ha, *va, *vh;
    const double *G, *rho;
    const double *drag_on, *drag_re, *drho, *drhod;
    const double* grav;
    double dt, m_h, kB, lim;
    const double* red2;
    double* dt_out;
    int first;
    double fixed_dt, dt_0, max_age;
    u64* counters;
};
__global__ __launch_bounds__(256) void dev_integrate_kernel(DevIntegArgs a) {
    int i = blockIdx.x * blockDim.x + threadIdx.x;
    if (i >= a.n) return;
    double dt = a.dt;
    if (a.red2) {
        if (a.red2[0] > 0.5) {
            if (i == 0) *a.dt_out = 0.0;
            return;
        }
        const double ct_min = -a.red2[1];
        const double ctv = sphx_ct_value(ct_min > DBL_MAX, ct_min, a.dt_0);
        dt = (a.fixed_dt > 0.0) ? a.fixed_dt : sphx_dt_rule(ctv, a.first, a.dt_0, a.max_age);
        if (i == 0) *a.dt_out = dt;
    }
    const double g = (a.ptype[i] == 0.0) ? 1.0 : 0.0;
    double v[3], pa[3], vis[3];
    bool bad_acc = false;
#pragma unroll
    for (int c = 0; c < 3; ++c) {
        v[c] = a.vel[3 * (size_t)i + c];
        if (a.G) {
            const double praw = a.G[3 * (size_t)i + c] / a.rho[i] * g;
            pa[c] = nan_to_num_v(praw);
            vis[c] = a.va[3 * (size_t)i + c];
            bad_acc = bad_acc || !sphx_finite(praw) || !sphx_finite(vis[c]);
        } else {
            const double praw = -a.ha[3 * (size_t)i + c] * g, vraw = -a.va[3 * (size_t)i + c] * g;
            pa[c] = nan_to_num_v(praw);
            vis[c] = nan_to_num_v(vraw);
            bad_acc = bad_acc || !sphx_finite(praw) || !sphx_finite(vraw);
        }
        if (a.drag_on) {
            const double draw = a.drag_on[3 * (size_t)i + c] * a.drhod[i] / a.drho[i] * g, rraw = a.drag_re[3 * (size_t)i + c];
            const double dg = nan_to_num_v(draw);
            vis[c] = dg + nan_to_num_v(rraw) + vis[c];
            bad_acc = bad_acc || !sphx_finite(draw) || !sphx_finite(rraw);
        }
    }
    double x[3], old[3], tot[3], gr[3] = {0.0, 0.0, 0.0};
#pragma unroll
    for (int c = 0; c < 3; ++c) { x[c] = a.pos[3 * (size_t)i + c]; old[c] = a.acc[3 * (size_t)i + c]; }
    if (a.grav)
#pragma unroll
        for (int c = 0; c < 3; ++c) gr[c] = a.grav[3 * (size_t)i + c];
    sphx_leapfrog_update(dt, x, v, vis, pa, a.grav ? gr : nullptr, old, tot);
#pragma unroll
    for (int c = 0; c < 3; ++c) {
        a.pos[3 * (size_t)i + c] = x[c];
        a.vel[3 * (size_t)i + c] = v[c];
        a.acc[3 * (size_t)i + c] = tot[c];
    }
    double E = a.E[i], T;
    const double heat = a.vh[i];
    const bool bad_en = !sphx_finite(E) || !sphx_finite(heat * dt);
    sphx_energy_update(dt, heat, a.mu[i], a.gam[i], a.m[i], a.m_h, a.kB, E, T);
    a.E[i] = E;
    a.T[i] = T;
    if (a.counters) {
        bool bad_st = false;
#pragma unroll
        for (int c = 0; c < 3; ++c) bad_st = bad_st || !sphx_finite(x[c]) || !sphx_finite(v[c]);
        sphx_count_bad(a.counters, BAD_ACCEL, bad_acc);
        sphx_count_bad(a.counters, BAD_ENERGY, bad_en);
        sphx_count_bad(a.counters, BAD_STATE, bad_st);
    }
}
static DevIntegArgs dev_integ_args(sphx_ctx* ctx, int64_t n_owned, double* pos, double* vel, double* accel_old, double* E_internal,
                                   double* T, const double* mass, const double* mu, const double* gamma, const double* ptype,
                                   const double* ha, const double* va, const double* vh, double dt) {
    DevIntegArgs a;
    a.n = (int)n_owned;
    a.pos = pos; a.vel = vel; a.acc = accel_old; a.E = E_internal; a.T = T;
    a.m = mass; a.mu = mu; a.gam = gamma; a.ptype = ptype;
    a.ha = ha; a.va = va; a.vh = vh;
    a.G = nullptr; a.rho = nullptr;
    a.drag_on = ctx->dev_drag_on; a.drag_re = ctx->dev_drag_re; a.drho = ctx->dev_drag_rho; a.drhod = ctx->dev_drag_rhod;
    ctx->dev_drag_on = ctx->dev_drag_re = ctx->dev_drag_rho = ctx->dev_drag_rhod = nullptr;
    a.grav = ctx->dev_grav;
    ctx->dev_grav = nullptr;
    a.dt = dt; a.m_h = ctx->cst.m_h; a.kB = ctx->cst.k_B; a.lim = ctx->cst.pos_clamp;
    a.red2 = nullptr; a.dt_out = nullptr; a.first = 0; a.fixed_dt = 0.0; a.dt_0 = ctx->cst.dt_0; a.max_age = ctx->cst.max_age;
    a.counters = ctx->badc.as<u64>();
    return a;
}
static int dev_integ_launch(sphx_ctx* ctx, const DevIntegArgs& a) {
    hipLaunchKernelGGL(dev_integrate_kernel, dim3((unsigned)((a.n + 255) / 256)), dim3(256), 0, ctx->stream, a);
    HIPCHK(hipGetLastError());
    return SPHX_OK;
}
__global__ __launch_bounds__(256) void dev_clamp_kernel(int n3, double lim, double* pos, double* vel) {
    int e = blockIdx.x * blockDim.x + threadIdx.x;
    if (e >= n3) return;
    pos[e] = sphx_clamp_pos(pos[e], lim);
    vel[e] = nan_to_num_v(vel[e]);
}

extern "C" int sphx_dev_clamp(sphx_ctx* ctx, int64_t n, double* pos, double* vel) {
    if (!ctx) return SPHX_E_ARG;
    NEED(pos); NEED(vel);
    HIPCHK(hipSetDevice(ctx->device));
    if (n < 1) return SPHX_OK;
    hipLaunchKernelGGL(dev_clamp_kernel, dim3((unsigned)((3 * n + 255) / 256)), dim3(256), 0, ctx->stream,
                       (int)(3 * n), ctx->cst.pos_clamp, pos, vel);
    HIPCHK(hipGetLastError());
    return SPHX_OK;
}

extern "C" int sphx_dev_integrate(sphx_ctx* ctx, int64_t n_owned, double* pos, double* vel, double* accel_old,
// ... 564 lines not shown
```

sph-code_amd/csrc/sphx_internal.h:

```cpp
#pragma once
#include <hip/hip_runtime.h>
#include <stdint.h>
#include <stdio.h>
#include <string.h>
#include <math.h>
#include <float.h>
#include <vector>
#include "../../include/sphx.h"
#include "sphx_agb.h"

#define SPHX_WAVE 64
#define SPHX_W6_C 1.5666814710608448

typedef unsigned long long u64;
typedef unsigned int u32;
struct PinnedLayout;

struct DevBuf {
    void* p = nullptr;
    size_t cap = 0;
    template <class T> T* as() const { return (T*)p; }
};

struct __attribute__((aligned(64))) RecA {
    double x, y, z;
    double h2;
    double c1;
    double ms;
    double A;
    double Nw;
};
struct __attribute__((aligned(64))) RecB {
    double x, y, z, h2;
    double vx, vy, vz;
    double cs;
};
struct __attribute__((aligned(16))) RecBC {
    double Bw;
    double c1;
};
struct __attribute__((aligned(32))) RecSelf {
    double csi;
    double h;
    double mg;
    double pad;
};

#define PYR_MAX 12
struct GravRef { double x, y, z; };
struct Pyr {
    int nlev;
    int nx[PYR_MAX + 1], ny[PYR_MAX + 1], nz[PYR_MAX + 1];
    long long off[PYR_MAX + 1];
};

struct GridParams {
    double xmin, ymin, zmin;
    double cell, inv_cell;
    int nx, ny, nz;
    int ncells;
    float fnx1, fny1, fnz1;
};

#define OLEV_N 32
#define OLEV_MAX 20
#define OLEV_MIN_RC 8.0f
struct OutLevels {
    int L;
    double cx, cy, cz;
    double hmax;
    const int* start;
    const int* list;
};
__device__ __forceinline__ bool sphx_outside_box(const GridParams& g, double x, double y, double z) {
    const double tx = (x - g.xmin) * g.inv_cell, ty = (y - g.ymin) * g.inv_cell, tz = (z - g.zmin) * g.inv_cell;
    return tx < 0.0 || tx >= (double)g.nx || ty < 0.0 || ty >= (double)g.ny || tz < 0.0 || tz >= (double)g.nz;
}

struct BlobBits { int bx, by, bz; int hilbert; };
__device__ __forceinline__ unsigned hilbert_rank(unsigned x, unsigned y, unsigned z, int b) {
    unsigned X[3] = {x, y, z};
    const unsigned M = 1u << (b - 1);
    for (unsigned Q = M; Q > 1; Q >>= 1) {
        const unsigned P = Q - 1;
#pragma unroll
        for (int i = 0; i < 3; ++i) {
            if (X[i] & Q) X[0] ^= P;
            else { const unsigned t = (X[0] ^ X[i]) & P; X[0] ^= t; X[i] ^= t; }
        }
    }
    X[1] ^= X[0]; X[2] ^= X[1];
    unsigned t = 0;
    for (unsigned Q = M; Q > 1; Q >>= 1)
        if (X[2] & Q) t ^= Q - 1;
    X[0] ^= t; X[1] ^= t; X[2] ^= t;
    unsigned out = 0;
    for (int q = 0; q < b; ++q) {
        out |= ((X[2] >> q) & 1u) << (3 * q);
        out |= ((X[1] >> q) & 1u) << (3 * q + 1);
        out |= ((X[0] >> q) & 1u) << (3 * q + 2);
    }
    return out;
}
__device__ __forceinline__ unsigned blob_rank(int cx, int cy, int cz, BlobBits b) {
    if (b.hilbert) return hilbert_rank((unsigned)cx, (unsigned)cy, (unsigned)cz, b.hilbert);
    unsigned out = 0;
    int pos = 0;
    for (int q = 0; q < 11; ++q) {
        if (q < b.bx) out |= (unsigned)((cx >> q) & 1) << pos++;
        if (q < b.by) out |= (unsigned)((cy >> q) & 1) << pos++;
        if (q < b.bz) out |= (unsigned)((cz >> q) & 1) << pos++;
    }
    return out;
}

struct StateArrays {
    DevBuf x, y, z, vx, vy, vz, ax, ay, az;
    DevBuf m, T, mu, gam, E, hprev;
    DevBuf ptype;
    DevBuf id;
    DevBuf fun;
    DevBuf mgm, mcs;
};

struct StageTimer {
    hipEvent_t ev[5] = {nullptr, nullptr, nullptr, nullptr, nullptr};
    double ms[4] = {0, 0, 0, 0};
    int begin(sphx_ctx* ctx);
    int mark(sphx_ctx* ctx, int i);
    int end(sphx_ctx* ctx);
};

#define SPHX_LDS_KERNELS 16

struct sphx_ctx {
    int device = 0;
    hipStream_t stream = nullptr;
    hipStream_t own_stream = nullptr;
    hipStream_t side_stream = nullptr;
    sphx_constants cst;
    char tunables[1024] = {0};
    double rscale = 1.08, cell_factor = 0.55;
    double rscale_build = 1.3;
    bool use_verlet = false;
    bool use_blob = true;
    int blob_curve = 0;
    bool use_group = true;
    bool use_lds = true;
    bool drag_lds = true;
    bool blob_split_on = true;
    bool species_lds = true;
    bool species_fused = true;
    int blob_grid = 0;
    int blob_slots = 1 << 20;
    int olev_mode = 2;
    int distrust_mode = 0;
    bool cell_feedback = true;
    double cell_fb_hi = 0.30, cell_fb_lo = 0.10;
    int64_t max_cells = 0;
    double box_sigmas = 3.0;
    double h_clip_factor = 8.0;
    double reach_cap = 0.0;
    bool timing_detail = false;
    int clip_grad = 0;
    int visc_mode = 0;
    bool drag = false;
    int loop_forms = 0;
    double loop_d = 0.0;
    int gravity = 0;
    double grav_G = 0.0;
    int grav_order = 2;
    bool grav_per_thread = false;
    int grav_ws = 1;
    bool agb_on = false;
    AgbTable agb;
    double dev_hmean = 0.0;

    char err[512] = {0};
    sphx_stats stats;
    int64_t n = 0, npad = 0;
    int k = 0, s = 0;
    int sp = 0;
    bool has_state = false;
    int64_t step_count = 0;
    double dt_last = 0.0;
    bool tprev_valid = false;
    bool ct_primed = false;
    bool recs_pw = false;
    bool nbr_api_valid = false;
    int64_t nbr_api_n = 0;
    int nbr_api_k = 0;
    bool list_valid = false;
    int64_t list_n = 0;
    int list_k = 0;
    const int* map_perm = nullptr;
    int map_nactive = 0;
    const int* qorder = nullptr;
    bool blob_lists = false;
    bool blob_split_valid = false;
    int blob_split_nblk = 0;
    int pass_part = 0;
    bool loop2_interior_done = false;
    bool dev_ev_pending = false;
    const double *dev_drag_on = nullptr, *dev_drag_re = nullptr, *dev_drag_rho = nullptr, *dev_drag_rhod = nullptr;
    const double* dev_grav = nullptr;
    bool gx_built = false;
    int64_t gx_n = 0, gx_nowned = 0;
    Pyr gx_py;
    GravRef gx_ref;
    GridParams grid;
    const double* tbox = nullptr;
    double tbox_h[6] = {0, 0, 0, 0, 0, 0};
    double clip_lo[3] = {0, 0, 0}, clip_hi[3] = {0, 0, 0};
    bool clip_valid = false;
    double h_clip = 0.0;
    double cell_scale = 1.0;
    bool cells_unsorted = false;
    bool curve_counted = false;
    bool order_by_count = false;
    bool blob_scatter_pending = false;
    BlobBits blob_scatter_bits;
    const int* blob_scatter_mstart = nullptr;
    bool bbox_ticket_zeroed = false;
    const void* cell_fill_zeroed = nullptr;
    const void* mcount_zeroed = nullptr;
    int mcount_zeroed_M = 0;
    const void* fcount_zeroed = nullptr;
    int64_t fcount_zeroed_n = 0;
    const void* tie_list_cleared = nullptr;
    const int* tie_count_dev = nullptr;
    int tie_cap_last = 0;
    const void* ds_cnt_zeroed = nullptr;
    const void* olev_fill_zeroed = nullptr;
    unsigned lbs_epoch[2] = {0u, 0u};
    const void* lds_raised[SPHX_LDS_KERNELS] = {nullptr};
    int n_lds_raised = 0;
    OutLevels olev;
    bool olev_ev_valid = false;
    u64 farq_seen = 0;
    int64_t farq_last = 0;
    int64_t list_len_last = 0;
    bool knn_lag_valid = false;
    u64 knn_lag[10] = {0, 0, 0, 0, 0, 0, 0, 0, 0, 0};
    u64 densep_seen = 0;
    int64_t densep_last = 0;
    u64 crowded_seen = 0;
    int64_t crowded_last = 0;
    bool distrust = false;
    u64 badhint_seen = 0;
    bool ev_detail[3] = {false, false, false};
    int ev_has07[3] = {0, 0, 0};
    unsigned ev_pending = 0;
    hipEvent_t lag_balias[2] = {nullptr, nullptr}, lag_halias[2] = {nullptr, nullptr};
    bool lag_bvalid[2] = {false, false}, lag_hvalid[2] = {false, false};
    int64_t lag_bn[2] = {0, 0};
    int lag_bslot = 0, lag_hslot = 0;

    std::vector<void*> allocs;
    DevBuf rec1, recv;
    DevBuf rho_s, bc_s, self_s;
    DevBuf drag_on, drag_re;
    DevBuf need_pyr;
    DevBuf fun_id;
    DevBuf crowded;
    DevBuf loop_side;
    DevBuf ds_cnt, ds_start, ds_ent;
    DevBuf lrec_a, lrec_v;
    DevBuf grav, grav_sort, grav_tmp;
    DevBuf grav_pyr, grav_cell;
    DevBuf grav_quad;
    DevBuf gx_pts, gx_m, gx_ord, gx_map, gx_box, gx_cflag, gx_coff, gx_pcnt, gx_poff, gx_counts;
    DevBuf list64, dref, pos0, pos4;
    DevBuf nbr;
    DevBuf porder, mcount, mstart;
    DevBuf agb_knots, Zmet, agb_dust;
    DevBuf fail_list;
    DevBuf olev_start, olev_fill, olev_list, olev_key;
    DevBuf lbs_state[2];
    DevBuf cell_rank;
    DevBuf perm_fin;
    DevBuf tie_list;
    DevBuf slot16, uniq;
    DevBuf blob_class, blob_split;
    DevBuf rho, rhod, nden, G, Pi, Bw, va, vh, ha, F;
    DevBuf scal;
    DevBuf cell_of, cell_start, cell_fill, perm, inv, scan_tmp, bbox_tmp;
    DevBuf in_a, in_b, in_c, in_d, in_e, in_f, in_g, in_h, in_i, in_j, out_a, out_b, out_c;
    DevBuf idx64, dist_out, nontriv, h_api;
    DevBuf arb_rec, arb_wrec, arb_flag, arb_cmax, arb_q, arb_key, arb_tmp, arb_acc, arb_out, arb_red;
    DevBuf arb_pos, arb_cs, arb_perm;
    int64_t arb_ball_id = 0, arb_ball_n = 0, arb_ball_m = 0;
    GridParams arb_g;
    double arb_tb[6] = {0, 0, 0, 0, 0, 0};
    StageTimer arb_t;
    DevBuf rad_in, rad_soa, rad_ray, rad_part, rad_gas, rad_out;
    StageTimer rad_t;
    DevBuf cool_in, cool_nb, cool_rec, cool_int, cool_rev, cool_tab, cool_out, cool_tmp;
    StageTimer cool_t;
    StateArrays st, alt;
    DevBuf badc;
    DevBuf scal_tmp;
    DevBuf hsum_tmp;
    hipEvent_t ev_join = nullptr;
    hipEvent_t ev_perm = nullptr;
    hipEvent_t olev_ev = nullptr;
    hipEvent_t ev[10] = {nullptr};
    hipEvent_t evring[3][10] = {{nullptr}};
    hipEvent_t lag_bev[2] = {nullptr, nullptr}, lag_hev[2] = {nullptr, nullptr};
    PinnedLayout* pinned = nullptr;
};

int sphx_set_err(sphx_ctx* ctx, int code, const char* fmt, ...);
int sphx_ensure(sphx_ctx* ctx, DevBuf& b, size_t bytes, hipStream_t in_use_on);
static inline int sphx_ensure(sphx_ctx* ctx, DevBuf& b, size_t bytes) { return sphx_ensure(ctx, b, bytes, ctx->stream); }
void sphx_release(sphx_ctx* ctx, DevBuf& b);

#define HIPCHK(expr)                                                                         \
    do {                                                                                     \
        hipError_t e_ = (expr);                                                              \
        if (e_ != hipSuccess)                                                                \
            return sphx_set_err(ctx, SPHX_E_HIP, "%s:%d %s -> %s", __FILE__, __LINE__,       \
                                #expr, hipGetErrorString(e_));                               \
    } while (0)
#define NEED(p)                                                                              \
    do {                                                                                     \
        if (!(p)) return sphx_set_err(ctx, SPHX_E_ARG, "%s: argument %s is NULL", __func__, #p); \
    } while (0)
#define SPHX_TRY(expr)                                                                       \
    do {                                                                                     \
        int r_ = (expr);                                                                     \
        if (r_ != SPHX_OK) return r_;                                                        \
    } while (0)

static inline int64_t sphx_pad64(int64_t n) { return (n + 63) & ~int64_t(63); }

__device__ __forceinline__ int xcd_block(int b, int nb) {
    const int q = nb >> 3, r = nb & 7, x = b & 7, s = b >> 3;
    return x * q + (x < r ? x : r) + s;
}

#ifndef SPHX_SUM_PARTS
#define SPHX_SUM_PARTS 4
#endif

__device__ __forceinline__ double sphx_nan_to_num(double v) {
    if (v != v) return 0.0;
    if (v > DBL_MAX) return DBL_MAX;
    if (v < -DBL_MAX) return -DBL_MAX;
    return v;
}

#define SPHX_CT_NONE 0x7FF0000000000000ull
int sphx_prime_ct(sphx_ctx* ctx, u64* ct_bits);

enum {
    SC_CT_BITS = 0,
    SC_DT = 1,
    SC_CAND = 2,
    SC_RETRY = 3,
    SC_HSUM = 4,
    SC_DISP2 = 5,
    SC_NFAIL = 6,
    SC_HCNT = 7,
    SC_GRAV_EPS = 8,
    SC_NFAILQ = 9,
    SC_SHORT = 10,
    SC_FARQ = 11,
    SC_BADHINT = 12,
    SC_CROWDED = 13,
    SC_DENSEP = 14,
    SC_KGDBG = 16,
    SC_SETTLED = 24,
    SC_NSLOTS = 26
};

enum {
    BAD_ACCEL = 0,
    BAD_ENERGY = 1,
    BAD_STATE = 2,
    BAD_H = 3,
    BADC_BUCKETS = 64, BADC_STRIDE = 16
};
int sphx_badc_read(sphx_ctx* ctx);

struct PinnedSide { double red[4]; int count; int pad_[7]; u64 cand; };
struct PinnedLag {
    double box[32];
    double hs[32];
};
struct PinnedLayout {
    union {
        u64 scal[SC_NSLOTS];
        PinnedSide side;
    };
    char pad0_[256 - SC_NSLOTS * 8];
    double hsum[4];
    char pad1_[1024 - 256 - 4 * 8];
    PinnedLag lag[2];
    char pad2_[3072 - 1024 - 2 * 512];
    u64 knn_lag[10];
    char pad3_[8192 - 3072 - 10 * 8];
    u64 badc[BADC_BUCKETS * BADC_STRIDE];
};
static_assert(sizeof(PinnedLayout) == 16384, "ctx->pinned is 16 KiB");
static_assert(offsetof(PinnedLayout, side) == 0 && offsetof(PinnedSide, count) == 32 && offsetof(PinnedSide, cand) == 64 &&
                  offsetof(PinnedLayout, hsum) == 256 && offsetof(PinnedLayout, lag) == 1024 && sizeof(PinnedLag) == 512 &&
                  offsetof(PinnedLag, hs) == 256 && offsetof(PinnedLayout, knn_lag) == 3072 && offsetof(PinnedLayout, badc) == 8192,
              "the offsets in use since the members were byte counts");
#define SPHX_PIN_APART(a, b) \
    static_assert(offsetof(PinnedLayout, a) + sizeof(PinnedLayout::a) <= offsetof(PinnedLayout, b), #a " overlaps " #b)
SPHX_PIN_APART(scal, hsum); SPHX_PIN_APART(side, hsum); SPHX_PIN_APART(hsum, lag); SPHX_PIN_APART(lag, knn_lag);
SPHX_PIN_APART(knn_lag, badc);
#undef SPHX_PIN_APART
static_assert(offsetof(PinnedLayout, badc) + sizeof(PinnedLayout::badc) == sizeof(PinnedLayout), "the buckets end the block");

struct CopyF64 { const void* host; const void* dev; size_t count; };
int sphx_upload_f64(sphx_ctx* ctx, const CopyF64* t, int nt);
int sphx_download_f64(sphx_ctx* ctx, const CopyF64* t, int nt);

int sphx_bbox(sphx_ctx* ctx, int64_t n, const double* x, const double* y, const double* z,
              double out_minmax[13], bool use_clip);
int sphx_median(sphx_ctx* ctx, int64_t n, const double* v, double* out_dev);
int sphx_gravity_launch(sphx_ctx* ctx, int64_t n, const double* x, const double* y, const double* z, int ps,
                        const double* m, const double* eps_dev, double eps, double G, const int* omap,
                        double* acc);
int sphx_gravity_tree_launch(sphx_ctx* ctx, int64_t n, const double* x, const double* y, const double* z,
                             const double* m, int ws, const double* eps_dev, double eps, double G, const int* omap,
                             double* acc);
int sphx_dev_collect(sphx_ctx* ctx);
int sphx_loop_step_sums(sphx_ctx* ctx, int64_t n, int k, double d);
int sphx_build_blob_order(sphx_ctx* ctx, int64_t n, bool defer_scatter = false);
static inline double sphx_cell_feedback(sphx_ctx* ctx, int64_t n) {
    if (ctx->cell_feedback && n > 0) {
        const double dense = (double)ctx->densep_last / (double)n;
        if (dense > ctx->cell_fb_hi) ctx->cell_scale = ctx->cell_scale * 0.97 > 0.35 ? ctx->cell_scale * 0.97 : 0.35;
        else if (dense < ctx->cell_fb_lo) ctx->cell_scale = ctx->cell_scale * 1.01 < 1.0 ? ctx->cell_scale * 1.01 : 1.0;
    }
    return ctx->cell_scale;
}
int sphx_blob_translate(sphx_ctx* ctx, int64_t n, int k);
int sphx_blob_density_species(sphx_ctx* ctx, int64_t n, int k, bool lean, int S, const double* fun, const int* row_of,
                              const double* m_sorted, double* F, double* Z, double* agb, int agb_on);
int sphx_blob_density(sphx_ctx* ctx, int64_t n, int k, bool lean);
int sphx_blob_pi(sphx_ctx* ctx, int64_t n, int k, u64* ct_bits);
int sphx_blob_visc(sphx_ctx* ctx, int64_t n, int k, const double* m);
int sphx_blob_visc_pw(sphx_ctx* ctx, int64_t n, int k, const double* m, u64* ct_bits);
int sphx_blob_species(sphx_ctx* ctx, int64_t n, int k, int S, const double* fun, const int* row_of, const double* m_sorted, double* F,
                      double* Z, double* agb, int agb_on);
#define CELL_SORT_SERIAL 16
#define CELL_SORT_WAVE 512
int sphx_cell_cues(sphx_ctx* ctx, hipStream_t stream);
struct OrderFinish {
    int n;
    GridParams g; BlobBits b;
    const int *perm_in, *cell_of, *cell_start, *mstart;
    int *perm_out, *porder, *mcount;
};
int sphx_finish_order_only(sphx_ctx* ctx, const OrderFinish& o);
struct GridBuildOpts {
    bool lagged = false;
    hipEvent_t alias_ev = nullptr;
    bool sort_cells_later = false;
    bool count_curve = false;
    double* clamp_vel[3] = {nullptr, nullptr, nullptr};
};
int sphx_build_grid(sphx_ctx* ctx, int64_t n, int k, const double* x, const double* y, const double* z, double cell_hint,
                    const GridBuildOpts& opts = GridBuildOpts());
struct GridHostState {
    GridParams grid;
    const double* tbox;
    double tbox_h[6], clip_lo[3], clip_hi[3], cell_size;
    bool clip_valid, cells_unsorted;
    int olev_L;
    int64_t cells;
    const int *map_perm, *qorder;
};
GridHostState sphx_grid_host_save(const sphx_ctx* ctx);
void sphx_grid_host_restore(sphx_ctx* ctx, const GridHostState& saved);
int sphx_excl_scan_int(sphx_ctx* ctx, const int* in, int* out, int n);
struct alignas(32) DragEntry { u64 key; double x, y, z; };
struct DragScatter { int* cnt; const int* start; DragEntry* ent; };
__device__ __forceinline__ void sphx_drag_put(const DragScatter& sc, int slot, u64 key, double x, double y, double z) {
    double2* q = reinterpret_cast<double2*>(sc.ent + slot);
    q[0] = make_double2(__longlong_as_double((long long)key), x);
    q[1] = make_double2(y, z);
}
int sphx_drag_scatter_plan(sphx_ctx* ctx, int64_t n, int k, const int* nbr, const double* ptype, const int* qorder, DragScatter* out,
                           bool blob = false);
int sphx_drag_scatter_reduce(sphx_ctx* ctx, int64_t n, const DragScatter& d, double* react);
int sphx_blob_drag(sphx_ctx* ctx, int64_t n, int k, bool count_only, const double* m, const double* ptype, const double* mgm,
                   const double* mcs, const int* id, double* onto, const DragScatter& sc);
int sphx_build_outlier_levels(sphx_ctx* ctx, int64_t n, const double* xs, const double* ys, const double* zs);
struct KnnIn {
    const double *xs, *ys, *zs;
    const int32_t* id;
    const int32_t* inv = nullptr;
    const double* rsearch = nullptr;
    double rscale = 1.0, rbound = 0.0;
    bool hinted = false;
    bool hint_by_id = false;
    bool lag_external = false;
};
struct KnnOut {
    int32_t* nbr;
    int32_t* list64 = nullptr;
    double* dref = nullptr;
    double* h_sorted;
    int64_t* idx64;
    double* dist;
    int64_t* nontriv;
    double* h_by_id;
};
int sphx_knn(sphx_ctx* ctx, int64_t n, int k, const KnnIn& in, const KnnOut& out);
struct PrepIn {
    const double *x, *y, *z; int ps;
    const double *vx, *vy, *vz; int vs;
    const double *m, *h, *T, *mu, *gam, *ptype;
    void pos_aos(const double* p) { x = p; y = p + 1; z = p + 2; ps = 3; }
    void vel_aos(const double* v) { vx = v; vy = v + 1; vz = v + 2; vs = 3; }
};
int sphx_prep(sphx_ctx* ctx, int64_t n, const PrepIn& in, bool pairwise, hipStream_t stream);
int sphx_pass_density(sphx_ctx* ctx, int64_t n, int k, bool lean = false);
int sphx_pass_pi(sphx_ctx* ctx, int64_t n, int k, const double* h, const double* ptype);
int sphx_pass_visc(sphx_ctx* ctx, int64_t n, int k, const double* m);
int sphx_pass_visc_pw(sphx_ctx* ctx, int64_t n, int k, const double* m);
int sphx_pass_species(sphx_ctx* ctx, int64_t n, int k, int s, const double* fun, double* F);
int sphx_step_species(sphx_ctx* ctx, int64_t n, int k);
int sphx_species_on(sphx_ctx* ctx, int64_t n, int k, int S, int SP, const double* fun, const int* row_of, const double* m_sorted,
                    double* F, double* Z, double* agb);
int sphx_agb_table_set(sphx_ctx* ctx, int S, int nspl, const int32_t* ntx, const int32_t* nty, const double* tx, const double* ty,
                       const double* coeffs, const int32_t* mapto, double divisor, const double* mu_specie, double solar_mass);
int sphx_transpose_nbr(sphx_ctx* ctx, int64_t n, int k, const int64_t* nb_rowmajor);

int sphx_clamp(sphx_ctx* ctx, int64_t n, StateArrays& s);
int sphx_permute_state(sphx_ctx* ctx, int64_t n, bool split, hipEvent_t after_first);
int sphx_hsum(sphx_ctx* ctx, int64_t n, const double* h, hipStream_t stream);
int sphx_compute_dt(sphx_ctx* ctx, int first, double fixed_dt);
int sphx_integrate(sphx_ctx* ctx, int64_t n, int fold_dt = 0, int first = 0, double fixed_dt = 0.0);
int sphx_pass_drag(sphx_ctx* ctx, int64_t n, int k, const double* m, const double* ptype, const double* mgm,
                   const double* mcs);
int sphx_aos_to_soa3(sphx_ctx* ctx, int64_t n, const double* aos, double* x, double* y, double* z);
int sphx_soa3_to_aos_by_id(sphx_ctx* ctx, int64_t n, const int* id, const double* x, const double* y,
                           const double* z, double* aos);
int sphx_scatter_rows_by_id(sphx_ctx* ctx, int64_t n, int w, const int* id, const double* in, double* out);
int sphx_gather3(sphx_ctx* ctx, int64_t n, const int* perm, const double* x, const double* y,
                 const double* z, double* xs, double* ys, double* zs);
int sphx_iota(sphx_ctx* ctx, int64_t n, int* out);
int sphx_knn_refresh(sphx_ctx* ctx, int64_t n, int k, const double* x, const double* y, const double* z,
                     int32_t* nbr, double* h_sorted, int64_t* nfail_out);
int sphx_save_list_positions(sphx_ctx* ctx, int64_t n, const double* x, const double* y, const double* z);
```

sph-code_amd/csrc/sphx_settled.h:

```cpp
#pragma once
#if defined(__HIPCC__)
#define SPHX_SETTLED_HD __host__ __device__
#else
#define SPHX_SETTLED_HD
#endif
SPHX_SETTLED_HD inline bool sphx_is_nan(double x) { return x != x; }
SPHX_SETTLED_HD inline bool sphx_row_settled(double own_bw, bool has_first, bool writes) {
    return writes && has_first && sphx_is_nan(own_bw);
}
SPHX_SETTLED_HD inline bool sphx_quad_saturated(bool s0, bool s1, bool s2, bool s3) { return (s0 || s1) || (s2 || s3); }
SPHX_SETTLED_HD inline bool sphx_wave_saturated(unsigned long long nan, unsigned long long live) {
    unsigned long long any = nan | (nan >> 1);
    any |= any >> 2;
    const unsigned long long first = 0x1111111111111111ull;
    return (live & first & ~any) == 0ull;
}
```

sph-code_amd/csrc/sphx_sums.hip:

```cpp
#include "sphx_internal.h"
#include "sphx_wave.h"
#include "sphx_pair.h"
#pragma clang fp contract(off)
#include <float.h>
#include <stdlib.h>

struct PrepArgs {
    int n;
    const double *x, *y, *z; int ps;
    const double *vx, *vy, *vz; int vs;
    const double *m, *h, *T, *mu, *gam, *ptype;
    double kB, amu;
    RecA* ra; RecB* rb; RecBC* bc; RecSelf* self;
    const int* perm;
    int which, n_active;
    int pairwise;
};

__global__ __launch_bounds__(256) void prep_kernel(PrepArgs a) {
    const int t = blockIdx.x * blockDim.x + threadIdx.x;
    if (t >= a.n) return;
    const int i = a.perm ? a.perm[t] : t;
    if (a.which && ((i < a.n_active) != (a.which == 1))) return;
    const double m = a.m[i], h = a.h[i], T = a.T[i], mu = a.mu[i], gam = a.gam[i], pt = a.ptype[i];
    const double g = (pt == 0.0) ? 1.0 : 0.0;
    RecA r; RecB v;
    r.x = a.x[(size_t)i * a.ps]; r.y = a.y[(size_t)i * a.ps]; r.z = a.z[(size_t)i * a.ps];
    const double h2 = h * h, h4 = h2 * h2, h8 = h4 * h4;
    r.h2 = h2;
    r.c1 = 315.0 / (201.06192982974676 * (h8 * h));
    r.ms = (pt == 0.0) ? m : ((pt == 2.0) ? -m : 0.0);
    const double nw = m / mu / a.amu;
    r.A = nw * a.kB * T * g;
    r.Nw = nw * g;
    v.x = r.x; v.y = r.y; v.z = r.z; v.h2 = h2;
    v.vx = a.vx[(size_t)i * a.vs]; v.vy = a.vy[(size_t)i * a.vs]; v.vz = a.vz[(size_t)i * a.vs];
    v.cs = sqrt(gam * a.kB * T / mu / a.amu * g);
    RecSelf sf;
    sf.csi = sqrt(gam * a.kB * T / (mu * a.amu) * g);
    sf.h = h; sf.mg = m * g; sf.pad = 0.0;
    RecBC bc; bc.Bw = a.pairwise ? sf.mg * r.c1 : 0.0; bc.c1 = r.c1;
    a.ra[t] = r;
    a.rb[t] = v;
    a.bc[t] = bc;
    a.self[t] = sf;
}

int sphx_prep(sphx_ctx* ctx, int64_t n, const PrepIn& in, bool pairwise, hipStream_t stream) {
    SPHX_TRY(sphx_ensure(ctx, ctx->rec1, (size_t)n * sizeof(RecA), stream));
    SPHX_TRY(sphx_ensure(ctx, ctx->recv, (size_t)n * sizeof(RecB), stream));
    SPHX_TRY(sphx_ensure(ctx, ctx->rho_s, (size_t)n * sizeof(double), stream));
    SPHX_TRY(sphx_ensure(ctx, ctx->bc_s, (size_t)n * sizeof(RecBC), stream));
    SPHX_TRY(sphx_ensure(ctx, ctx->self_s, (size_t)n * sizeof(RecSelf), stream));
    PrepArgs a;
    a.n = (int)n;
    a.x = in.x; a.y = in.y; a.z = in.z; a.ps = in.ps;
    a.vx = in.vx; a.vy = in.vy; a.vz = in.vz; a.vs = in.vs;
    a.m = in.m; a.h = in.h; a.T = in.T; a.mu = in.mu; a.gam = in.gam; a.ptype = in.ptype;
    a.kB = ctx->cst.k_B; a.amu = ctx->cst.amu;
    a.ra = ctx->rec1.as<RecA>();
    a.rb = ctx->recv.as<RecB>();
    a.bc = ctx->bc_s.as<RecBC>();
    a.self = ctx->self_s.as<RecSelf>();
    a.perm = ctx->map_perm;
    a.which = ctx->map_perm ? ctx->pass_part : 0;
    a.n_active = ctx->map_nactive;
    a.pairwise = pairwise ? 1 : 0;
    ctx->recs_pw = pairwise;
    hipLaunchKernelGGL(prep_kernel, dim3((unsigned)((n + 255) / 256)), dim3(256), 0, stream, a);
    HIPCHK(hipGetLastError());
    return SPHX_OK;
}

__global__ __launch_bounds__(256) void transpose_nbr_kernel(long long n, int k, int npad,
                                                            const long long* nb, int* out) {
    long long e = (long long)blockIdx.x * blockDim.x + threadIdx.x;
    if (e >= n * k) return;
    long long i = e / k;
    int kk = (int)(e - i * k);
    long long j = nb[e];
    out[(long long)kk * npad + i] = (j >= 0 && j < n) ? (int)j : -1;
}

int sphx_transpose_nbr(sphx_ctx* ctx, int64_t n, int k, const int64_t* nb_dev) {
    int64_t npad = sphx_pad64(n);
    SPHX_TRY(sphx_ensure(ctx, ctx->nbr, (size_t)k * npad * sizeof(int)));
    HIPCHK(hipMemsetAsync(ctx->nbr.p, 0xFF, (size_t)k * npad * sizeof(int), ctx->stream));
    long long tot = (long long)n * k;
    hipLaunchKernelGGL(transpose_nbr_kernel, dim3((unsigned)((tot + 255) / 256)), dim3(256), 0,
                       ctx->stream, (long long)n, k, (int)npad, (const long long*)nb_dev,
                       ctx->nbr.as<int>());
    HIPCHK(hipGetLastError());
    return SPHX_OK;
}

struct OutMap { const int* perm; int n_active; };
__device__ __forceinline__ int out_index(const OutMap& m, int i) { return m.perm ? m.perm[i] : i; }

#define NBATCH 4

__global__ __launch_bounds__(256) void pass_density_kernel(int n, int npad, int k, int clip,
                                                           const int* __restrict__ nbr,
                                                           const RecA* __restrict__ rec, double* rho_s,
                                                           const int* __restrict__ qorder, OutMap om, double* rho,
                                                           double* rhod, double* nden, double* G,
                                                           double* ha) {
    const int p = xcd_block(blockIdx.x, gridDim.x) * blockDim.x + threadIdx.x;
    if (p >= n) return;
    const int i = qorder ? qorder[p] : p;
    const int o = out_index(om, i);
    if (o >= om.n_active) return;
    const double* self = reinterpret_cast<const double*>(&rec[i]);
    const Q4 s0 = gload4(self), s1 = gload4(self + 4);
    int j0 = nbr[p];
    double xr = s0.a, yr = s0.b, zr = s0.c;
    if (j0 >= 0 && j0 != i) { xr = rec[j0].x; yr = rec[j0].y; zr = rec[j0].z; }
    const double hi2 = s0.d, ci = -6.0 * s1.a, Ai = s1.c;
    DensAcc acc[SPHX_SUM_PARTS] = {};
    for (int kk0 = 0; kk0 < k; kk0 += NBATCH) {
      int jb[NBATCH];
      Q4 q0b[NBATCH], q1b[NBATCH];
#pragma unroll
      for (int u = 0; u < NBATCH; ++u) jb[u] = (kk0 + u < k) ? nbr[(size_t)(kk0 + u) * npad + p] : -1;
#pragma unroll
      for (int u = 0; u < NBATCH; ++u) {
          const double* q = reinterpret_cast<const double*>(&rec[jb[u] < 0 ? i : jb[u]]);
          q0b[u] = gload4(q); q1b[u] = gload4(q + 4);
      }
#pragma unroll
      for (int u = 0; u < NBATCH; ++u) {
        if (jb[u] < 0) continue;
        density_term<SqrtLib>(acc[u & (SPHX_SUM_PARTS - 1)], q0b[u], q1b[u], xr, yr, zr, hi2, ci, Ai, clip != 0);
      }
    }
    const double s_rho = parts_total(acc, &DensAcc::rho), s_rd = parts_total(acc, &DensAcc::rd), s_n = parts_total(acc, &DensAcc::n);
    const double gx = parts_total(acc, &DensAcc::gx), gy = parts_total(acc, &DensAcc::gy), gz = parts_total(acc, &DensAcc::gz);
    rho[o] = s_rho; rhod[o] = s_rd; nden[o] = s_n;
    rho_s[i] = s_rho;
    if (G) { G[3 * (size_t)o + 0] = -gx; G[3 * (size_t)o + 1] = -gy; G[3 * (size_t)o + 2] = -gz; }
    ha[3 * (size_t)o + 0] = -gx / s_rho;
    ha[3 * (size_t)o + 1] = -gy / s_rho;
    ha[3 * (size_t)o + 2] = -gz / s_rho;
}

int sphx_pass_density(sphx_ctx* ctx, int64_t n, int k, bool lean) {
    SPHX_TRY(sphx_ensure(ctx, ctx->rho, (size_t)n * sizeof(double)));
    SPHX_TRY(sphx_ensure(ctx, ctx->rhod, (size_t)n * sizeof(double)));
    SPHX_TRY(sphx_ensure(ctx, ctx->nden, (size_t)n * sizeof(double)));
    SPHX_TRY(sphx_ensure(ctx, ctx->G, (size_t)n * 3 * sizeof(double)));
    SPHX_TRY(sphx_ensure(ctx, ctx->ha, (size_t)n * 3 * sizeof(double)));
    if (ctx->qorder && ctx->blob_lists) return sphx_blob_density(ctx, n, k, lean);
    hipLaunchKernelGGL(pass_density_kernel, dim3((unsigned)((n + 255) / 256)), dim3(256), 0, ctx->stream,
                       (int)n, (int)sphx_pad64(n), k, ctx->clip_grad, ctx->nbr.as<int>(), ctx->rec1.as<RecA>(),
                       ctx->rho_s.as<double>(), ctx->qorder, OutMap{ctx->map_perm, ctx->map_perm ? ctx->map_nactive : (int)n},
                       ctx->rho.as<double>(), ctx->rhod.as<double>(), ctx->nden.as<double>(),
                       lean ? nullptr : ctx->G.as<double>(), ctx->ha.as<double>());
    HIPCHK(hipGetLastError());
    return SPHX_OK;
}

__global__ __launch_bounds__(256) void pass_pi_kernel(int n, int npad, int k, const int* __restrict__ nbr,
                                                      const RecB* __restrict__ recb,
                                                      const double* __restrict__ rho_s,
                                                      const RecSelf* __restrict__ selfr, RecBC* bc,
                                                      const int* __restrict__ qorder, OutMap om, double* Pi, double* BwOut,
                                                      u64* ct_bits) {
    const int p = xcd_block(blockIdx.x, gridDim.x) * blockDim.x + threadIdx.x;
    u64 my_ct = SPHX_CT_NONE;
    const int i = (p < n) ? (qorder ? qorder[p] : p) : n;
    const int o = (i < n) ? out_index(om, i) : 0x7FFFFFFF;
    if (i < n && o < om.n_active) {
        int j0 = nbr[p];
        if (j0 < 0) j0 = i;
        const double* rq = reinterpret_cast<const double*>(&recb[j0]);
        const Q4 r0 = gload4(rq), rv = gload4(rq + 4);
        const RecSelf sf = selfr[i];
        const double rho_i = rho_s[i], cs_i = sf.csi, ms_i = sf.mg, h_i = sf.h;
        double a_pi[SPHX_SUM_PARTS] = {}, maxrel = 0.0;
        for (int kk0 = 0; kk0 < k; kk0 += NBATCH) {
          int jb[NBATCH];
          Q4 q0b[NBATCH], qvb[NBATCH];
          double rhob[NBATCH];
#pragma unroll
          for (int u = 0; u < NBATCH; ++u) jb[u] = (kk0 + u < k) ? nbr[(size_t)(kk0 + u) * npad + p] : -1;
#pragma unroll
          for (int u = 0; u < NBATCH; ++u) {
              const int jj = jb[u] < 0 ? i : jb[u];
              const double* qb = reinterpret_cast<const double*>(&recb[jj]);
              q0b[u] = gload4(qb); qvb[u] = gload4(qb + 4);
              rhob[u] = rho_s[jj];
          }
#pragma unroll
          for (int u = 0; u < NBATCH; ++u) {
            if (jb[u] < 0) continue;
            const PiPair t = pi_term<SqrtLib>(q0b[u], qvb[u], rhob[u], r0, rv, rho_i, cs_i);
            a_pi[u & (SPHX_SUM_PARTS - 1)] += t.pi;
            maxrel = fmax(maxrel, t.rel);
          }
        }
        const double s_pi = parts_total(a_pi);
        Pi[o] = s_pi;
        const double bw = fmax(ms_i, 0.0) * s_pi;
        bc[i].Bw = bw;
        if (BwOut) BwOut[o] = bw;
        if (ms_i > 0.0) my_ct = ct_vote_bits(h_i, maxrel);
    }
    block_min_vote<256>(my_ct, ct_bits);
}

int sphx_pass_pi(sphx_ctx* ctx, int64_t n, int k, const double* h, const double* ptype) {
    (void)ptype; (void)h;
    SPHX_TRY(sphx_ensure(ctx, ctx->Pi, (size_t)n * sizeof(double)));
    SPHX_TRY(sphx_ensure(ctx, ctx->Bw, (size_t)n * sizeof(double)));
    u64* ct = ctx->scal.as<u64>() + SC_CT_BITS;
    if (!ctx->ct_primed) SPHX_TRY(sphx_prime_ct(ctx, ct));
    ctx->ct_primed = false;
    if (ctx->qorder && ctx->blob_lists) return sphx_blob_pi(ctx, n, k, ct);
    hipLaunchKernelGGL(pass_pi_kernel, dim3((unsigned)((n + 255) / 256)), dim3(256), 0, ctx->stream,
                       (int)n, (int)sphx_pad64(n), k, ctx->nbr.as<int>(), ctx->recv.as<RecB>(),
                       ctx->rho_s.as<double>(), ctx->self_s.as<RecSelf>(), ctx->bc_s.as<RecBC>(), ctx->qorder,
                       OutMap{ctx->map_perm, ctx->map_perm ? ctx->map_nactive : (int)n},
                       ctx->Pi.as<double>(), ctx->map_perm ? ctx->Bw.as<double>() : nullptr, ct);
    HIPCHK(hipGetLastError());
    return SPHX_OK;
}

__global__ __launch_bounds__(256) void pass_visc_kernel(int n, int npad, int k, int clip,
                                                        const int* __restrict__ nbr,
                                                        const RecB* __restrict__ recb,
                                                        const RecBC* __restrict__ bc,
                                                        const int* __restrict__ qorder, OutMap om,
                                                        const double* __restrict__ m, double* va,
                                                        double* vh) {
    const int p = xcd_block(blockIdx.x, gridDim.x) * blockDim.x + threadIdx.x;
    if (p >= n) return;
    const int i = qorder ? qorder[p] : p;
    const int o = out_index(om, i);
    if (o >= om.n_active) return;
    int j0 = nbr[p];
    if (j0 < 0) j0 = i;
    const double* rq = reinterpret_cast<const double*>(&recb[j0]);
    const Q4 r0 = gload4(rq), rv = gload4(rq + 4);
    const double2 bci = *reinterpret_cast<const double2*>(&bc[i]);
    const double hi2 = recb[i].h2, ci = -6.0 * bci.y, Bi = bci.x;
    ViscAcc acc[SPHX_SUM_PARTS] = {};
    for (int kk0 = 0; kk0 < k; kk0 += NBATCH) {
      int jb[NBATCH];
      Q4 q0b[NBATCH], qvb[NBATCH];
      double2 bcb[NBATCH];
#pragma unroll
      for (int u = 0; u < NBATCH; ++u) jb[u] = (kk0 + u < k) ? nbr[(size_t)(kk0 + u) * npad + p] : -1;
#pragma unroll
      for (int u = 0; u < NBATCH; ++u) {
          const int jj = jb[u] < 0 ? i : jb[u];
          const double* qb = reinterpret_cast<const double*>(&recb[jj]);
          q0b[u] = gload4(qb); qvb[u] = gload4(qb + 4);
          bcb[u] = *reinterpret_cast<const double2*>(&bc[jj]);
      }
#pragma unroll
      for (int u = 0; u < NBATCH; ++u) {
        if (jb[u] < 0) continue;
        visc_term<SqrtLib>(acc[u & (SPHX_SUM_PARTS - 1)], q0b[u], qvb[u], bcb[u].x, bcb[u].y, r0, rv, hi2, ci, Bi, clip != 0);
      }
    }
    const double ax = parts_total(acc, &ViscAcc::x), ay = parts_total(acc, &ViscAcc::y), az = parts_total(acc, &ViscAcc::z);
    const double heat = parts_total(acc, &ViscAcc::h);
    va[3 * (size_t)o + 0] = -ax; va[3 * (size_t)o + 1] = -ay; va[3 * (size_t)o + 2] = -az;
    vh[o] = heat * m[o] / 2.0;
}

int sphx_pass_visc(sphx_ctx* ctx, int64_t n, int k, const double* m) {
    SPHX_TRY(sphx_ensure(ctx, ctx->va, (size_t)n * 3 * sizeof(double)));
    SPHX_TRY(sphx_ensure(ctx, ctx->vh, (size_t)n * sizeof(double)));
    if (ctx->qorder && ctx->blob_lists) return sphx_blob_visc(ctx, n, k, m);
    hipLaunchKernelGGL(pass_visc_kernel, dim3((unsigned)((n + 255) / 256)), dim3(256), 0, ctx->stream,
                       (int)n, (int)sphx_pad64(n), k, ctx->clip_grad, ctx->nbr.as<int>(), ctx->recv.as<RecB>(),
                       ctx->bc_s.as<RecBC>(), ctx->qorder,
                       OutMap{ctx->map_perm, ctx->map_perm ? ctx->map_nactive : (int)n}, m,
                       ctx->va.as<double>(), ctx->vh.as<double>());
    HIPCHK(hipGetLastError());
    return SPHX_OK;
}

__global__ __launch_bounds__(256) void pass_visc_pw_kernel(int n, int npad, int k, int clip,
                                                           const int* __restrict__ nbr,
                                                           const RecB* __restrict__ recb,
                                                           const double* __restrict__ rho_s,
                                                           const RecBC* __restrict__ bc,
                                                           const RecSelf* __restrict__ selfr,
                                                           const int* __restrict__ qorder, OutMap om,
                                                           const double* __restrict__ m, double* va, double* vh,
                                                           u64* ct_bits) {
    const int p = xcd_block(blockIdx.x, gridDim.x) * blockDim.x + threadIdx.x;
    u64 my_ct = SPHX_CT_NONE;
    const int i = (p < n) ? (qorder ? qorder[p] : p) : n;
    const int o = (i < n) ? out_index(om, i) : 0x7FFFFFFF;
    if (i < n && o < om.n_active) {
        int j0 = nbr[p];
        if (j0 < 0) j0 = i;
        const double* rq = reinterpret_cast<const double*>(&recb[j0]);
        const Q4 r0 = gload4(rq), rv = gload4(rq + 4);
        const RecSelf sf = selfr[i];
        const double rho_i = rho_s[i], cs_i = sf.csi, h_i = sf.h;
        const double hi2 = recb[i].h2, ci = -6.0 * bc[i].Bw;
        ViscAcc acc[SPHX_SUM_PARTS] = {};
        double maxrel = 0.0;
        for (int kk0 = 0; kk0 < k; kk0 += NBATCH) {
          int jb[NBATCH];
          Q4 q0b[NBATCH], qvb[NBATCH];
          double rhob[NBATCH], mcb[NBATCH];
#pragma unroll
          for (int u = 0; u < NBATCH; ++u) jb[u] = (kk0 + u < k) ? nbr[(size_t)(kk0 + u) * npad + p] : -1;
#pragma unroll
          for (int u = 0; u < NBATCH; ++u) {
              const int jj = jb[u] < 0 ? i : jb[u];
              const double* qb = reinterpret_cast<const double*>(&recb[jj]);
              q0b[u] = gload4(qb); qvb[u] = gload4(qb + 4);
              rhob[u] = rho_s[jj];
              mcb[u] = bc[jj].Bw;
          }
#pragma unroll
          for (int u = 0; u < NBATCH; ++u) {
            if (jb[u] < 0) continue;
            maxrel = fmax(maxrel, visc_pw_term<SqrtLib>(acc[u & (SPHX_SUM_PARTS - 1)], q0b[u], qvb[u], rhob[u], mcb[u], r0, rv,
                                                         rho_i, cs_i, hi2, ci, clip != 0));
          }
        }
        const double ax = parts_total(acc, &ViscAcc::x), ay = parts_total(acc, &ViscAcc::y), az = parts_total(acc, &ViscAcc::z);
        const double heat = parts_total(acc, &ViscAcc::h);
        va[3 * (size_t)o + 0] = -ax; va[3 * (size_t)o + 1] = -ay; va[3 * (size_t)o + 2] = -az;
        vh[o] = heat * m[o] / 2.0;
        if (sf.mg > 0.0) my_ct = ct_vote_bits(h_i, maxrel);
    }
    block_min_vote<256>(my_ct, ct_bits);
}

int sphx_pass_visc_pw(sphx_ctx* ctx, int64_t n, int k, const double* m) {
    SPHX_TRY(sphx_ensure(ctx, ctx->va, (size_t)n * 3 * sizeof(double)));
    SPHX_TRY(sphx_ensure(ctx, ctx->vh, (size_t)n * sizeof(double)));
    u64* ct = ctx->scal.as<u64>() + SC_CT_BITS;
    if (!ctx->ct_primed) SPHX_TRY(sphx_prime_ct(ctx, ct));
    ctx->ct_primed = false;
    if (ctx->qorder && ctx->blob_lists) return sphx_blob_visc_pw(ctx, n, k, m, ct);
    hipLaunchKernelGGL(pass_visc_pw_kernel, dim3((unsigned)((n + 255) / 256)), dim3(256), 0, ctx->stream,
                       (int)n, (int)sphx_pad64(n), k, ctx->clip_grad, ctx->nbr.as<int>(), ctx->recv.as<RecB>(),
                       ctx->rho_s.as<double>(), ctx->bc_s.as<RecBC>(), ctx->self_s.as<RecSelf>(), ctx->qorder,
                       OutMap{ctx->map_perm, ctx->map_perm ? ctx->map_nactive : (int)n}, m,
                       ctx->va.as<double>(), ctx->vh.as<double>(), ct);
    HIPCHK(hipGetLastError());
    return SPHX_OK;
}

__global__ __launch_bounds__(256) void drag_count_kernel(int n, int npad, int k, const int* __restrict__ nbr,
                                                         const double* __restrict__ ptype, const int* __restrict__ qorder,
                                                         int* cnt) {
    const int p = blockIdx.x * blockDim.x + threadIdx.x;
    if (p >= n) return;
    const int i = qorder ? qorder[p] : p;
    for (int kk = 0; kk < k; ++kk) {
        const int j = nbr[(size_t)kk * npad + p];
        if (j >= 0 && j != i && ptype[j] == 2.0) atomicAdd(&cnt[j], 1);
    }
}
#define DRAG_RED_BLOCKS 2048
#define DRAG_RED_U 4
template <int U>
__device__ __forceinline__ void drag_slice_sum(int s, int L, const DragEntry* __restrict__ ent,
                                               double* pk, int lane, double& acc) {
    u64 key[U];
    double vx[U], vy[U], vz[U];
// ... 287 lines not shown
```

Before: 944.7 million.

## Precompute per-blob settled flags in Pi pass so visc pass skips settled blobs

The Pi blob pass now works out, per blob, whether every row is settled or inactive. It writes a byte flag per blob and pre-fills NaN viscosity outputs for settled rows. The visc blob pass reads these flags with one wave-wide ballot per 64 blob iterations and skips flagged blobs without staging, replacing the old per-blob lookahead and extra barrier vote. A fallback flags kernel runs when the Pi pass did not mark. This adds NaN writes and a flag store to the Pi pass in exchange for less visc-pass overhead.

Result: no change. 948.4 million, median of 6 (+0.4%).

```diff
diff --git a/sph-code_amd/csrc/sphx_api.hip b/sph-code_amd/csrc/sphx_api.hip
--- a/sph-code_amd/csrc/sphx_api.hip
+++ b/sph-code_amd/csrc/sphx_api.hip
@@ -116,6 +116,7 @@
     if (const char* e = env("SPHX_CELL_FB_LO")) ctx->cell_fb_lo = atof(e);
     if (const char* e = env("SPHX_DRAG_LDS")) ctx->drag_lds = atoi(e) != 0;
     if (const char* e = env("SPHX_BLOB_SPLIT")) ctx->blob_split_on = atoi(e) != 0;
+    if (const char* e = env("SPHX_VISC_MARK")) ctx->visc_mark = atoi(e) != 0;
     if (const char* e = env("SPHX_SPECIES_FUSED")) ctx->species_fused = atoi(e) != 0;
     if (const char* e = env("SPHX_SPECIES_LDS")) ctx->species_lds = atoi(e) != 0;
     if (const char* e = env("SPHX_HINT_DISTRUST")) ctx->distrust_mode = atoi(e);
@@ -667,7 +668,13 @@
         if (ctx->visc_mode == 1) {
             SPHX_TRY(sphx_pass_visc_pw(ctx, n, k, s.m.as<double>()));
         } else {
-            SPHX_TRY(sphx_pass_pi(ctx, n, k, s.hprev.as<double>(), s.ptype.as<double>()));
+            const bool mark = ctx->visc_mark && ctx->qorder && ctx->blob_lists;
+            if (mark) {
+                SPHX_TRY(sphx_ensure(ctx, ctx->va, (size_t)n * 3 * sizeof(double)));
+                SPHX_TRY(sphx_ensure(ctx, ctx->vh, (size_t)n * sizeof(double)));
+            }
+            SPHX_TRY(sphx_pass_pi(ctx, n, k, s.hprev.as<double>(), s.ptype.as<double>(), mark));
+            ctx->visc_flags_valid = mark;
             if (detail) HIPCHK(hipEventRecord(ev[5], ctx->stream));
             SPHX_TRY(sphx_pass_visc(ctx, n, k, s.m.as<double>()));
         }
@@ -689,6 +696,7 @@
     ctx->qorder = nullptr;
     ctx->blob_lists = false;
     ctx->blob_split_valid = false;
+    ctx->visc_flags_valid = false;
     ctx->pass_part = 0;
     ctx->nbr_api_valid = false;
     if (rec0) HIPCHK(hipEventRecord(ev[0], ctx->stream));
diff --git a/sph-code_amd/csrc/sphx_blob.h b/sph-code_amd/csrc/sphx_blob.h
--- a/sph-code_amd/csrc/sphx_blob.h
+++ b/sph-code_amd/csrc/sphx_blob.h
@@ -179,6 +179,8 @@
 
 template <class P, class = void> struct BlobSettles { static constexpr bool value = false; };
 template <class P> struct BlobSettles<P, decltype((void)P::SETTLES)> { static constexpr bool value = P::SETTLES; };
+template <class P, class = void> struct BlobMarks { static constexpr bool value = false; };
+template <class P> struct BlobMarks<P, decltype((void)P::MARKS)> { static constexpr bool value = P::MARKS; };
 template <class P, class = void> struct BlobSaturates { static constexpr bool value = false; };
 template <class P> struct BlobSaturates<P, decltype((void)P::SATURATES)> { static constexpr bool value = P::SATURATES; };
 enum { BLOB_CNT_BLOBS_SETTLED = 0, BLOB_CNT_WAVES_SATURATED = 1 };
@@ -243,17 +245,6 @@
         out[u] = P::term_short(f[u], row);
     }
 }
-struct RowAhead { int i, o; unsigned first; double own; };
-template <class P>
-__device__ __forceinline__ RowAhead blob_row_ahead(const P& ps, int i, int p, int n, const u16* __restrict__ slot16,
-                                                   const int* __restrict__ omap) {
-    RowAhead r;
-    r.i = i;
-    r.o = (p < n) ? (omap ? omap[i] : i) : 0x7FFFFFFF;
-    r.first = (p < n) ? slot16[p] : SLOT_NONE;
-    r.own = ps.own(i);
-    return r;
-}
 template <int T>
 __device__ __forceinline__ bool block_all_at_barrier(bool mine, unsigned round) {
     __shared__ int verdict[2][T / 64];
@@ -292,7 +283,7 @@
                                           const int* __restrict__ qorder, int clip, const int* __restrict__ omap,
                                           int n_active, u64* ct_bits, const BlobSel& sel, u64* counts = nullptr) {
     static_assert(P::PER_SLOT == 64 + (P::NSIDE ? 8 : 0), "image bytes per slot: the record and one side value");
-    constexpr bool SETTLES = BlobSettles<P>::value, SATURATES = BlobSaturates<P>::value;
+    constexpr bool SETTLES = BlobSettles<P>::value, SATURATES = BlobSaturates<P>::value, MARKS = BlobMarks<P>::value;
     static_assert(!SATURATES || LPP == 4, "sphx_wave_saturated: a row's lanes are one nibble of the wave's mask");
     typedef BlobLds<P::NSIDE> L;
     const BlobSides sd = ps.sides();
@@ -301,57 +292,34 @@
     unsigned blobs_settled = 0, waves_saturated = 0;
     const int nsel = blob_sel_count(sel, nblk);
     const int stride = gridDim.x;
-    auto particle_of = [&](int bq) -> int {
-        const int pq = blob_sel_at(sel, bq, nsel) * BLOB_P + t;
-        return (pq < n) ? qorder[pq] : 0;
-    };
-    auto nothing_left = [&](const RowAhead& r) -> bool {
-        return !(r.o < n_active) || sphx_row_settled(r.own, r.first != SLOT_NONE, true);
-    };
-    RowAhead cur{0, 0x7FFFFFFF, SLOT_NONE, 0.0};
-    int i_next = 0;
-    bool blob_settled = false;
+    unsigned step = 0;
+    u64 flagged = 0;
     unsigned round = 0;
-    if constexpr (SETTLES) {
-        if ((int)blockIdx.x < nsel)
-            cur = blob_row_ahead(ps, particle_of(blockIdx.x), blob_sel_at(sel, blockIdx.x, nsel) * BLOB_P + t, n, slot16, omap);
-        if ((int)blockIdx.x + stride < nsel) i_next = particle_of(blockIdx.x + stride);
-        blob_settled = block_all_at_barrier<PASS_T>(nothing_left(cur), round++);
-    }
     for (int bi = blockIdx.x; bi < nsel; bi += stride) {
+        if constexpr (SETTLES) {
+            if (sphx_flag_refill_due(step)) {
+                const long long w = sphx_flag_lane_position(bi, stride, threadIdx.x & 63u);
+                bool f = false;
+                if (sphx_flag_in_selection(w, nsel)) f = ps.flags[blob_sel_at(sel, (int)w, nsel)] != 0;
+                flagged = __ballot(f);
+            }
+            const bool skip = (flagged >> sphx_flag_bit(step)) & 1ull;
+            ++step;
+            if (skip) { ++blobs_settled; continue; }
+        }
         const int b = blob_sel_at(sel, bi, nsel);
         const int p = b * BLOB_P + t;
-        int i, o;
-        bool settled = false;
-        auto fetch_ahead = [&]() {
-            if constexpr (SETTLES) {
-                if (bi + stride < nsel) {
-                    cur = blob_row_ahead(ps, i_next, blob_sel_at(sel, bi + stride, nsel) * BLOB_P + t, n, slot16, omap);
-                    if (bi + 2 * stride < nsel) i_next = particle_of(bi + 2 * stride);
-                }
-            }
-        };
-        if constexpr (SETTLES) {
-            i = cur.i; o = cur.o;
-            settled = sphx_row_settled(cur.own, cur.first != SLOT_NONE, o < n_active);
-            if (blob_settled) {
-                fetch_ahead();
-                if (settled && !half) ps.settle(o);
-                ++blobs_settled;
-                blob_settled = block_all_at_barrier<PASS_T>(nothing_left(cur), round++);
-                continue;
-            }
-        } else {
-            i = (p < n) ? qorder[p] : 0;
-        }
+        const int i = (p < n) ? qorder[p] : 0;
         stage<P::NSIDE>(L::img(), L::side(), L::tile(), ps.rec, sd.g0, sd.s0, sd.g1, sd.s1, uniq + (size_t)b * BLOB_S,
                         slot16, npad, k, b);
         typename P::Row row = ps.load_row(i);
-        if constexpr (!SETTLES) o = (p < n) ? (omap ? omap[i] : i) : 0x7FFFFFFF;
+        const int o = (p < n) ? (omap ? omap[i] : i) : 0x7FFFFFFF;
         ps.load_out(row, o, o < n_active);
-        if constexpr (SETTLES) fetch_ahead();
         __syncthreads();
+        bool nothing_left = true;
         if (o < n_active) {
+            bool settled = false;
+            if constexpr (SETTLES) settled = sphx_row_settled(P::own(row), L::tile()[t] != SLOT_NONE, true);
             if (SETTLES && __ballot(!settled) == 0ull) {
                 if constexpr (SETTLES) { if (!half) ps.settle(o); }
             } else {
@@ -393,13 +361,19 @@
                 group_total_fields(a);
                 if (P::VOTES) mx = group_max(mx);
                 if (!half) {
-                    const u64 cb = ps.finish(a, mx, row, i, o);
+                    u64 cb;
+                    if constexpr (MARKS) cb = ps.finish(a, mx, row, i, o, L::tile()[t] != SLOT_NONE, n_active, nothing_left);
+                    else cb = ps.finish(a, mx, row, i, o);
                     my_ct = cb < my_ct ? cb : my_ct;
                 }
             }
         }
-        if constexpr (SETTLES) blob_settled = block_all_at_barrier<PASS_T>(nothing_left(cur), round++);
-        else __syncthreads();
+        if constexpr (MARKS) {
+            const bool all = block_all_at_barrier<PASS_T>(nothing_left, round++);
+            if (ps.flags && threadIdx.x == 0) ps.flags[b] = all ? 1 : 0;
+        } else {
+            __syncthreads();
+        }
     }
     if (P::VOTES) block_min_vote<PASS_T>(my_ct, ct_bits);
     if constexpr (SETTLES) {
diff --git a/sph-code_amd/csrc/sphx_blob.hip b/sph-code_amd/csrc/sphx_blob.hip
--- a/sph-code_amd/csrc/sphx_blob.hip
+++ b/sph-code_amd/csrc/sphx_blob.hip
@@ -168,6 +168,8 @@
     const int nblk = (int)((npad + BLOB_P - 1) / BLOB_P);
     SPHX_TRY(sphx_ensure(ctx, ctx->slot16, (size_t)k * npad * sizeof(u16) + 512));
     SPHX_TRY(sphx_ensure(ctx, ctx->uniq, (size_t)nblk * BLOB_S * sizeof(int)));
+    SPHX_TRY(sphx_ensure(ctx, ctx->visc_flags, (size_t)nblk));
+    ctx->visc_flags_valid = false;
     int slots = ctx->blob_slots;
     if (slots < 1) slots = 1;
     if (slots > BLOB_S) slots = BLOB_S;
@@ -243,11 +245,14 @@
     static constexpr int NSIDE = 1, PER_SLOT = 72;
     static constexpr bool CLIPS = false, VOTES = true, ROW_FROM_LIST = true;
     static constexpr bool SATURATES = BLOB_PI_SATURATES != 0;
+    static constexpr bool MARKS = true;
     const RecB* __restrict__ rec;
     const double* __restrict__ rho_s;
     const RecSelf* __restrict__ selfr;
     RecBC* bc;
     double *Pi, *BwOut;
+    double *va, *vh;
+    unsigned char* flags;
     struct Row { Q4 r0, rv; double rho_i, cs_i, ms_i, h_i; };
     struct Nb { Q8 q; double rho; };
     __device__ __forceinline__ BlobSides sides() const { return {rho_s, 1}; }
@@ -276,18 +281,26 @@
     __device__ __forceinline__ Vel short_global(int j) const { return gload4(reinterpret_cast<const double*>(&rec[j]) + 4); }
     __device__ __forceinline__ static Vel short_none(const Row& r) { return r.rv; }
     __device__ __forceinline__ static double term_short(const Vel& qv, const Row& r) { return pi_rel(qv, r.rv); }
-    __device__ __forceinline__ u64 finish(const Sums& a, double maxrel, const Row& r, int i, int o) const {
+    __device__ __forceinline__ u64 finish(const Sums& a, double maxrel, const Row& r, int i, int o, bool has_first,
+                                          int n_active, bool& left) const {
         Pi[o] = a.pi;
         const double bw = fmax(r.ms_i, 0.0) * a.pi;
         bc[i].Bw = bw;
         if (BwOut) BwOut[o] = bw;
+        left = sphx_row_nothing_left(bw, has_first, o, n_active);
+        if (flags && sphx_row_settled(bw, has_first, o < n_active)) {
+            const double q = __builtin_nan("");
+            va[3 * (size_t)o + 0] = q; va[3 * (size_t)o + 1] = q; va[3 * (size_t)o + 2] = q;
+            vh[o] = q;
+        }
         return (r.ms_i > 0.0) ? ct_vote_bits(r.h_i, maxrel) : SPHX_CT_NONE;
     }
 };
 BLOB_KERNEL blob_pi_kernel(BLOB_COMMON, const int* __restrict__ omap, int n_active, const RecB* __restrict__ recb,
                            const double* __restrict__ rho_s, const RecSelf* __restrict__ selfr, RecBC* bc, double* Pi,
-                           double* BwOut, u64* ct_bits, BlobSel sel, u64* counts) {
-    blob_pass(PiPass{recb, rho_s, selfr, bc, Pi, BwOut}, n, npad, k, nblk, nbr, slot16, uniq, qorder, 0, omap, n_active,
+                           double* BwOut, double* va, double* vh, unsigned char* flags, u64* ct_bits, BlobSel sel,
+                           u64* counts) {
+    blob_pass(PiPass{recb, rho_s, selfr, bc, Pi, BwOut, va, vh, flags}, n, npad, k, nblk, nbr, slot16, uniq, qorder, 0, omap, n_active,
               ct_bits, sel, counts);
 }
 
@@ -301,6 +314,7 @@
     const RecBC* __restrict__ bc;
     const double* __restrict__ m;
     double *va, *vh;
+    const unsigned char* __restrict__ flags;
     struct Row { Q4 r0, rv; double hi2, ci, Bi, mi; };
     struct Nb { Q8 q; double c1; };
     __device__ __forceinline__ BlobSides sides() const {
@@ -335,7 +349,7 @@
         vh[o] = a.h * r.mi / 2.0;
         return SPHX_CT_NONE;
     }
-    __device__ __forceinline__ double own(int i) const { return bc[i].Bw; }
+    __device__ __forceinline__ static double own(const Row& r) { return r.Bi; }
     __device__ __forceinline__ void settle(int o) const {
         const double q = __builtin_nan("");
         va[3 * (size_t)o + 0] = q; va[3 * (size_t)o + 1] = q; va[3 * (size_t)o + 2] = q;
@@ -344,9 +358,36 @@
 };
 BLOB_KERNEL blob_visc_kernel(BLOB_COMMON, int clip, const int* __restrict__ omap, int n_active,
                              const RecB* __restrict__ recb, const RecBC* __restrict__ bc, const double* __restrict__ m,
-                             double* va, double* vh, BlobSel sel, u64* counts) {
-    blob_pass(ViscPass{recb, bc, m, va, vh}, n, npad, k, nblk, nbr, slot16, uniq, qorder, clip, omap, n_active, nullptr, sel,
+                             double* va, double* vh, const unsigned char* __restrict__ flags, BlobSel sel, u64* counts) {
+    blob_pass(ViscPass{recb, bc, m, va, vh, flags}, n, npad, k, nblk, nbr, slot16, uniq, qorder, clip, omap, n_active, nullptr, sel,
               counts);
+}
+
+__global__ __launch_bounds__(BLOB_P) void blob_flags_kernel(int n, int nblk, const u16* __restrict__ slot16,
+                                                            const int* __restrict__ qorder, const int* __restrict__ omap,
+                                                            int n_active, const RecBC* __restrict__ bc, double* va,
+                                                            double* vh, unsigned char* flags, BlobSel sel) {
+    const int nsel = blob_sel_count(sel, nblk);
+    if ((int)blockIdx.x >= nsel) return;
+    const int b = blob_sel_at(sel, blockIdx.x, nsel);
+    const int p = b * BLOB_P + threadIdx.x;
+    int o = 0x7FFFFFFF;
+    double bw = 0.0;
+    bool has_first = false;
+    if (p < n) {
+        const int i = qorder[p];
+        o = omap ? omap[i] : i;
+        bw = bc[i].Bw;
+        has_first = slot16[p] != SLOT_NONE;
+    }
+    const bool settled = sphx_row_settled(bw, has_first, o < n_active);
+    const int all = __syncthreads_and(sphx_row_nothing_left(bw, has_first, o, n_active) ? 1 : 0);
+    if (threadIdx.x == 0) flags[b] = all ? 1 : 0;
+    if (all && settled) {
+        const double q = __builtin_nan("");
+        va[3 * (size_t)o + 0] = q; va[3 * (size_t)o + 1] = q; va[3 * (size_t)o + 2] = q;
+        vh[o] = q;
+    }
 }
 
 struct ViscPwPass {
@@ -723,17 +764,28 @@
                        sphx_blob_sel(ctx, ctx->pass_part));
 }
 
-int sphx_blob_pi(sphx_ctx* ctx, int64_t n, int k, u64* ct_bits) {
+int sphx_blob_pi(sphx_ctx* ctx, int64_t n, int k, u64* ct_bits, bool mark) {
     return blob_launch(ctx, blob_pi_kernel, PiPass::PER_SLOT, 0, n, k, ctx->map_perm, blob_n_active(ctx, n), ctx->recv.as<RecB>(),
                        ctx->rho_s.as<double>(), ctx->self_s.as<RecSelf>(), ctx->bc_s.as<RecBC>(), ctx->Pi.as<double>(),
-                       ctx->map_perm ? ctx->Bw.as<double>() : nullptr, ct_bits, sphx_blob_sel(ctx, ctx->pass_part),
+                       ctx->map_perm ? ctx->Bw.as<double>() : nullptr, mark ? ctx->va.as<double>() : nullptr,
+                       mark ? ctx->vh.as<double>() : nullptr, mark ? ctx->visc_flags.as<unsigned char>() : nullptr, ct_bits,
+                       sphx_blob_sel(ctx, ctx->pass_part), ctx->scal.as<u64>() + SC_SETTLED);
+}
+
+int sphx_blob_visc(sphx_ctx* ctx, int64_t n, int k, const double* m) {
+    const BlobSel sel = sphx_blob_sel(ctx, ctx->pass_part);
+    unsigned char* flags = ctx->visc_flags.as<unsigned char>();
+    if (!ctx->visc_flags_valid) {
+        const int nblk = (int)((sphx_pad64(n) + BLOB_P - 1) / BLOB_P);
+        hipLaunchKernelGGL(blob_flags_kernel, dim3(nblk), dim3(BLOB_P), 0, ctx->stream, (int)n, nblk, ctx->slot16.as<u16>(),
+                           ctx->qorder, ctx->map_perm, blob_n_active(ctx, n), ctx->bc_s.as<RecBC>(), ctx->va.as<double>(),
+                           ctx->vh.as<double>(), flags, sel);
+        HIPCHK(hipGetLastError());
+    }
+    ctx->visc_flags_valid = false;
+    return blob_launch(ctx, blob_visc_kernel, ViscPass::PER_SLOT, 0, n, k, ctx->clip_grad, ctx->map_perm, blob_n_active(ctx, n),
+                       ctx->recv.as<RecB>(), ctx->bc_s.as<RecBC>(), m, ctx->va.as<double>(), ctx->vh.as<double>(), flags, sel,
                        ctx->scal.as<u64>() + SC_SETTLED);
-}
-
-int sphx_blob_visc(sphx_ctx* ctx, int64_t n, int k, const double* m) {
-    return blob_launch(ctx, blob_visc_kernel, ViscPass::PER_SLOT, 0, n, k, ctx->clip_grad, ctx->map_perm, blob_n_active(ctx, n),
-                       ctx->recv.as<RecB>(), ctx->bc_s.as<RecBC>(), m, ctx->va.as<double>(), ctx->vh.as<double>(),
-                       sphx_blob_sel(ctx, ctx->pass_part), ctx->scal.as<u64>() + SC_SETTLED);
 }
 
 int sphx_blob_visc_pw(sphx_ctx* ctx, int64_t n, int k, const double* m, u64* ct_bits) {
diff --git a/sph-code_amd/csrc/sphx_dev.hip b/sph-code_amd/csrc/sphx_dev.hip
--- a/sph-code_amd/csrc/sphx_dev.hip
+++ b/sph-code_amd/csrc/sphx_dev.hip
@@ -81,6 +81,7 @@
     ctx->qorder = nullptr;
     ctx->blob_lists = false;
     ctx->blob_split_valid = false;
+    ctx->visc_flags_valid = false;
     ctx->pass_part = 0;
     if (ctx->use_blob) SPHX_TRY(sphx_build_blob_order(ctx, n));
     ctx->map_nactive = (int)n_owned;
@@ -209,6 +210,7 @@
         hipLaunchKernelGGL(inject_field_kernel, dim3((unsigned)((n + 255) / 256)), dim3(256), 0, ctx->stream, (int)n,
                            ctx->map_perm, Bw_complete, ctx->bc_s.as<double>(), 2);
     HIPCHK(hipGetLastError());
+    ctx->visc_flags_valid = false;
     Borrow b1(ctx->va, visc_accel, 3 * (size_t)n * sizeof(double)), b2(ctx->vh, visc_heat, (size_t)n * sizeof(double));
     SPHX_TRY(sphx_pass_visc(ctx, n, ctx->k, mass));
     return SPHX_OK;
diff --git a/sph-code_amd/csrc/sphx_internal.h b/sph-code_amd/csrc/sphx_internal.h
--- a/sph-code_amd/csrc/sphx_internal.h
+++ b/sph-code_amd/csrc/sphx_internal.h
@@ -149,6 +149,7 @@
     bool use_lds = true;
     bool drag_lds = true;
     bool blob_split_on = true;
+    bool visc_mark = true;
     bool species_lds = true;
     bool species_fused = true;
     int blob_grid = 0;
@@ -198,6 +199,7 @@
     const int* qorder = nullptr;
     bool blob_lists = false;
     bool blob_split_valid = false;
+    bool visc_flags_valid = false;
     int blob_split_nblk = 0;
     int pass_part = 0;
     bool loop2_interior_done = false;
@@ -281,6 +283,7 @@
     DevBuf perm_fin;
     DevBuf tie_list;
     DevBuf slot16, uniq;
+    DevBuf visc_flags;
     DevBuf blob_class, blob_split;
     DevBuf rho, rhod, nden, G, Pi, Bw, va, vh, ha, F;
     DevBuf scal;
@@ -442,7 +445,7 @@
 int sphx_blob_density_species(sphx_ctx* ctx, int64_t n, int k, bool lean, int S, const double* fun, const int* row_of,
                               const double* m_sorted, double* F, double* Z, double* agb, int agb_on);
 int sphx_blob_density(sphx_ctx* ctx, int64_t n, int k, bool lean);
-int sphx_blob_pi(sphx_ctx* ctx, int64_t n, int k, u64* ct_bits);
+int sphx_blob_pi(sphx_ctx* ctx, int64_t n, int k, u64* ct_bits, bool mark);
 int sphx_blob_visc(sphx_ctx* ctx, int64_t n, int k, const double* m);
 int sphx_blob_visc_pw(sphx_ctx* ctx, int64_t n, int k, const double* m, u64* ct_bits);
 int sphx_blob_species(sphx_ctx* ctx, int64_t n, int k, int S, const double* fun, const int* row_of, const double* m_sorted, double* F,
@@ -521,7 +524,7 @@
 };
 int sphx_prep(sphx_ctx* ctx, int64_t n, const PrepIn& in, bool pairwise, hipStream_t stream);
 int sphx_pass_density(sphx_ctx* ctx, int64_t n, int k, bool lean = false);
-int sphx_pass_pi(sphx_ctx* ctx, int64_t n, int k, const double* h, const double* ptype);
+int sphx_pass_pi(sphx_ctx* ctx, int64_t n, int k, const double* h, const double* ptype, bool mark = false);
 int sphx_pass_visc(sphx_ctx* ctx, int64_t n, int k, const double* m);
 int sphx_pass_visc_pw(sphx_ctx* ctx, int64_t n, int k, const double* m);
 int sphx_pass_species(sphx_ctx* ctx, int64_t n, int k, int s, const double* fun, double* F);
diff --git a/sph-code_amd/csrc/sphx_settled.h b/sph-code_amd/csrc/sphx_settled.h
--- a/sph-code_amd/csrc/sphx_settled.h
+++ b/sph-code_amd/csrc/sphx_settled.h
@@ -15,3 +15,17 @@
     const unsigned long long first = 0x1111111111111111ull;
     return (live & first & ~any) == 0ull;
 }
+
+SPHX_SETTLED_HD inline bool sphx_row_nothing_left(double own_bw, bool has_first, int o, int n_active) {
+    return !(o < n_active) || sphx_row_settled(own_bw, has_first, true);
+}
+enum { SPHX_FLAG_MASK_BITS = 64 };
+SPHX_SETTLED_HD inline bool sphx_flag_refill_due(unsigned step) { return (step & (SPHX_FLAG_MASK_BITS - 1)) == 0u; }
+SPHX_SETTLED_HD inline unsigned sphx_flag_bit(unsigned step) { return step & (SPHX_FLAG_MASK_BITS - 1); }
+SPHX_SETTLED_HD inline long long sphx_flag_position(int first, int stride, unsigned refill, unsigned bit) {
+    return (long long)first + ((long long)refill * SPHX_FLAG_MASK_BITS + bit) * (long long)stride;
+}
+SPHX_SETTLED_HD inline long long sphx_flag_lane_position(int at, int stride, unsigned lane) {
+    return (long long)at + (long long)lane * (long long)stride;
+}
+SPHX_SETTLED_HD inline bool sphx_flag_in_selection(long long position, int nsel) { return position < (long long)nsel; }
diff --git a/sph-code_amd/csrc/sphx_sums.hip b/sph-code_amd/csrc/sphx_sums.hip
--- a/sph-code_amd/csrc/sphx_sums.hip
+++ b/sph-code_amd/csrc/sphx_sums.hip
@@ -52,6 +52,7 @@
     SPHX_TRY(sphx_ensure(ctx, ctx->rho_s, (size_t)n * sizeof(double), stream));
     SPHX_TRY(sphx_ensure(ctx, ctx->bc_s, (size_t)n * sizeof(RecBC), stream));
     SPHX_TRY(sphx_ensure(ctx, ctx->self_s, (size_t)n * sizeof(RecSelf), stream));
+    ctx->visc_flags_valid = false;
     PrepArgs a;
     a.n = (int)n;
     a.x = in.x; a.y = in.y; a.z = in.z; a.ps = in.ps;
@@ -208,14 +209,15 @@
     block_min_vote<256>(my_ct, ct_bits);
 }
 
-int sphx_pass_pi(sphx_ctx* ctx, int64_t n, int k, const double* h, const double* ptype) {
+int sphx_pass_pi(sphx_ctx* ctx, int64_t n, int k, const double* h, const double* ptype, bool mark) {
     (void)ptype; (void)h;
+    ctx->visc_flags_valid = false;
     SPHX_TRY(sphx_ensure(ctx, ctx->Pi, (size_t)n * sizeof(double)));
     SPHX_TRY(sphx_ensure(ctx, ctx->Bw, (size_t)n * sizeof(double)));
     u64* ct = ctx->scal.as<u64>() + SC_CT_BITS;
     if (!ctx->ct_primed) SPHX_TRY(sphx_prime_ct(ctx, ct));
     ctx->ct_primed = false;
-    if (ctx->qorder && ctx->blob_lists) return sphx_blob_pi(ctx, n, k, ct);
+    if (ctx->qorder && ctx->blob_lists) return sphx_blob_pi(ctx, n, k, ct, mark);
     hipLaunchKernelGGL(pass_pi_kernel, dim3((unsigned)((n + 255) / 256)), dim3(256), 0, ctx->stream,
                        (int)n, (int)sphx_pad64(n), k, ctx->nbr.as<int>(), ctx->recv.as<RecB>(),
                        ctx->rho_s.as<double>(), ctx->self_s.as<RecSelf>(), ctx->bc_s.as<RecBC>(), ctx->qorder,
```
